# D-Robotics/hobot_stereonet

Hardware: AMD Instinct MI355X
Metric: stereo pairs/s at 1280x720 D=192 (ms/frame alongside) (higher is better)
Workload: dtype f16 (refinement-tower MFMA operands fp16 — 3x3 weights rounded per kernel so that every kernel's tap sum survives —, LeakyReLU applied after the fp16 rounding; low-resolution branch on 22-bit hi/lo split fp16 operands, 3 fp16 MFMAs per product in every 32-channel layer — profiles/r04_lowres_ablation

## Files before the change

hobot_stereonet_amd/api.py:

```python
from __future__ import annotations

import ctypes as C
import os
from typing import Optional

import numpy as np

from . import build as _build

SN_MEM_HOST, SN_MEM_DEVICE = 0, 1
PREC_DEFAULT, PREC_F16X3, PREC_F16, PREC_FP32, PREC_AUTO = 0, 1, 2, 3, 4
PREC_NAMES = {PREC_F16X3: "f16x3", PREC_F16: "f16", PREC_FP32: "fp32", PREC_AUTO: "auto"}
ABI_VERSION = 3
STAGES = ("features", "aggregate", "refine", "refine_conv", "total", "dominant")


class SnConfig(C.Structure):
    _fields_ = [("device", C.c_int), ("max_batch", C.c_int), ("width", C.c_int), ("height", C.c_int),
                ("dmax", C.c_int), ("precision", C.c_int), ("task_num", C.c_int), ("refine_chunk", C.c_int),
                ("piece", C.c_int)]


class SnIoInfo(C.Structure):
    _fields_ = [("width", C.c_int), ("height", C.c_int), ("dmax", C.c_int), ("in_channels", C.c_int),
                ("max_batch", C.c_int), ("precision", C.c_int), ("task_num", C.c_int), ("device", C.c_int),
                ("out_scale", C.c_float), ("in_bytes", C.c_size_t), ("out_bytes", C.c_size_t),
                ("flops_per_pair", C.c_double), ("refine_chunk", C.c_int), ("piece", C.c_int),
                ("tower_streams", C.c_int), ("refine_levels", C.c_int), ("precision_selected", C.c_int)]


class SnRefineStats(C.Structure):
    _fields_ = [("levels", C.c_int), ("precision", C.c_int), ("precision_selected", C.c_int), ("precision_last", C.c_int),
                ("calls", C.c_uint64), ("pairs", C.c_uint64), ("switches", C.c_uint64), ("reruns", C.c_uint64),
                ("level_px", C.c_double * 4), ("residual_px", C.c_double), ("running_px", C.c_double),
                ("envelope_px", C.c_double), ("limit_px", C.c_double), ("selfcheck_epe_px", C.c_double),
                ("selfcheck_residual_px", C.c_double)]


class SnAutoState(C.Structure):
    _fields_ = [("mode", C.c_int), ("calm", C.c_int), ("envelope_px", C.c_double), ("epe_per_px", C.c_double),
                ("running_px", C.c_double), ("switches", C.c_uint64)]


class StereoNetError(RuntimeError):
    def __init__(self, code: int, where: str, detail: str = ""):
        self.code = code
        super().__init__(f"{where}: {error_string(code)} (code {code}){': ' + detail if detail else ''}")


_lib = None


def load_library(path: Optional[str] = None):
    global _lib
    if _lib is not None:
        return _lib
    path = path or os.environ.get("STEREONET_HIP_LIB") or _build.LIB
    try:
        import torch
    except ImportError:
        pass
    if not os.path.exists(path) or (os.path.exists(_build.HIPCC) and _build.is_stale()):
        _build.build()
    lib = C.CDLL(path)
    vp, ip, i8p, i32p, fp, u8p = C.c_void_p, C.c_int, C.c_void_p, C.c_void_p, C.c_void_p, C.c_void_p
    lib.sn_create.argtypes = [C.c_char_p, C.POINTER(SnConfig), C.POINTER(vp)]
    lib.sn_destroy.argtypes = [vp]
    lib.sn_get_io_info.argtypes = [vp, C.POINTER(SnIoInfo)]
    lib.sn_strerror.restype = C.c_char_p
    lib.sn_strerror.argtypes = [ip]
    lib.sn_last_error.restype = C.c_char_p
    lib.sn_last_error.argtypes = [vp]
    lib.sn_infer_i8.argtypes = [vp, i8p, i32p, fp, ip, vp]
    lib.sn_infer_batch.argtypes = [vp, ip, i8p, i32p, fp, ip, vp]
    lib.sn_preprocess_nv12.argtypes = [vp, u8p, u8p, ip, ip, i8p, ip, vp]
    lib.sn_infer_sbs_nv12.argtypes = [vp, u8p, ip, ip, i32p, fp, i8p, ip, vp]
    lib.sn_preprocess_sbs_nv12_batch.argtypes = [vp, ip, u8p, ip, ip, i8p, ip, vp]
    lib.sn_submit.argtypes = [vp, i8p, i32p, fp, ip, C.POINTER(C.c_uint64)]
    lib.sn_submit_nv12.argtypes = [vp, u8p, ip, ip, i32p, fp, ip, C.POINTER(C.c_uint64)]
    lib.sn_wait.argtypes = [vp, C.c_uint64, C.POINTER(C.c_float)]
    lib.sn_synchronize.argtypes = [vp]
    lib.sn_set_profiling.argtypes = [vp, ip]
    lib.sn_get_stage_ms.argtypes = [vp, C.POINTER(C.c_float), ip]
    lib.sn_get_dominant_kernel.argtypes = [vp, C.c_char_p, C.c_size_t, C.POINTER(ip), C.POINTER(C.c_double),
                                           C.POINTER(C.c_double)]
    lib.sn_mgpu_shard.argtypes = [ip, ip, ip, C.POINTER(ip), C.POINTER(ip)]
    lib.sn_mgpu_create.argtypes = [C.c_char_p, C.POINTER(SnConfig), C.POINTER(ip), ip, C.POINTER(vp)]
    lib.sn_mgpu_destroy.argtypes = [vp]
    lib.sn_mgpu_get_info.argtypes = [vp, C.POINTER(ip), C.POINTER(ip), C.POINTER(ip)]
    lib.sn_mgpu_get_handle.argtypes = [vp, ip, C.POINTER(vp)]
    lib.sn_mgpu_infer_batch.argtypes = [vp, ip, i8p, i32p, fp]
    lib.sn_mgpu_infer_batch_device.argtypes = [vp, ip, C.POINTER(vp), i32p, fp]
    lib.sn_mgpu_submit_device.argtypes = [vp, ip, C.POINTER(vp), i32p, fp, C.POINTER(C.c_uint64)]
    lib.sn_mgpu_wait.argtypes = [vp, C.c_uint64]
    lib.sn_mgpu_ring_init.argtypes = [vp]
    lib.sn_mgpu_ring_submit.argtypes = [vp, C.POINTER(C.c_uint64), C.POINTER(ip)]
    lib.sn_mgpu_ring_wait.argtypes = [vp, C.c_uint64, C.POINTER(ip)]
    lib.sn_mgpu_last_error.restype = C.c_char_p
    lib.sn_mgpu_last_error.argtypes = [vp]
    lib.sn_dbg_conv2d.argtypes = [vp, fp, ip, ip, ip, fp, fp, ip, ip, ip, ip, fp, fp]
    lib.sn_dbg_down0.argtypes = [vp, i8p, ip, ip, fp, fp, ip, fp]
    lib.sn_dbg_compose_down01.argtypes = [fp, fp, fp, fp, fp, fp]
    lib.sn_dbg_round_kernels_f16.argtypes = [fp, ip, fp]
    lib.sn_dbg_down01.argtypes = [vp, i8p, ip, ip, fp, fp, fp, fp, fp]
    lib.sn_dbg_refin.argtypes = [vp, fp, i8p, ip, ip, ip, fp, fp, ip, fp]
    lib.sn_dbg_conv3d.argtypes = [vp, fp, ip, ip, ip, fp, fp, ip, fp]
    lib.sn_dbg_ref_conv_f16.argtypes = [vp, fp, ip, ip, fp, fp, ip, ip, fp, fp]
    lib.sn_dbg_ref_conv_f16x3.argtypes = [vp, fp, ip, ip, fp, fp, ip, ip, fp, fp]
    lib.sn_dbg_ref_block_f16.argtypes = [vp, fp, ip, ip, fp, fp, fp, fp, ip, fp]
    lib.sn_dbg_ref_block_f16x3.argtypes = [vp, fp, ip, ip, fp, fp, fp, fp, ip, ip, fp]
    lib.sn_dbg_ref_tail_f16.argtypes = [vp, ip, fp, ip, ip, fp, fp, fp, fp, fp, C.c_float, fp, ip, C.c_float, ip, ip, ip, fp, i32p]
    lib.sn_dbg_read.argtypes = [vp, C.c_char_p, fp, C.c_size_t, C.POINTER(C.c_size_t)]
    lib.sn_dbg_copy_limited.argtypes = [vp, vp, C.c_size_t, ip, vp]
    lib.sn_depth_from_raw.argtypes = [vp, ip, i32p, C.c_float, C.c_float, fp, fp, ip, vp]
    lib.sn_get_refine_stats.argtypes = [vp, C.POINTER(SnRefineStats)]
    lib.sn_auto_init.argtypes = [C.POINTER(SnAutoState), ip]
    lib.sn_auto_observe.argtypes = [C.POINTER(SnAutoState), C.c_double]
    lib.sn_auto_limit_px.argtypes = [C.POINTER(SnAutoState)]
    lib.sn_auto_limit_px.restype = C.c_double
    lib.sn_auto_envelope_px.argtypes = [ip]
    lib.sn_auto_envelope_px.restype = C.c_double
    for name in ("sn_create", "sn_destroy", "sn_get_io_info", "sn_infer_i8", "sn_infer_batch", "sn_preprocess_nv12",
                 "sn_infer_sbs_nv12", "sn_preprocess_sbs_nv12_batch", "sn_submit", "sn_submit_nv12", "sn_wait", "sn_synchronize", "sn_set_profiling",
                 "sn_get_stage_ms", "sn_get_dominant_kernel", "sn_mgpu_shard", "sn_mgpu_create", "sn_mgpu_destroy",
                 "sn_mgpu_get_info", "sn_mgpu_get_handle", "sn_mgpu_infer_batch", "sn_mgpu_infer_batch_device",
                 "sn_mgpu_submit_device", "sn_mgpu_wait", "sn_mgpu_ring_init", "sn_mgpu_ring_submit", "sn_mgpu_ring_wait", "sn_dbg_conv2d", "sn_dbg_down0", "sn_dbg_compose_down01", "sn_dbg_round_kernels_f16", "sn_dbg_down01", "sn_dbg_refin", "sn_dbg_conv3d", "sn_dbg_ref_conv_f16", "sn_dbg_ref_conv_f16x3", "sn_dbg_ref_block_f16", "sn_dbg_ref_block_f16x3", "sn_dbg_ref_tail_f16", "sn_dbg_read", "sn_dbg_copy_limited", "sn_depth_from_raw", "sn_get_refine_stats", "sn_auto_init", "sn_auto_observe"):
        getattr(lib, name).restype = C.c_int
    _lib = lib
    return lib


def round_kernels_f16(w):
    a = np.ascontiguousarray(w, np.float32)
    assert a.shape[-2:] == (3, 3)
    out = np.empty_like(a)
    rc = load_library().sn_dbg_round_kernels_f16(a.ctypes.data, a.size // 9, out.ctypes.data)
    if rc:
        raise StereoNetError(rc, "sn_dbg_round_kernels_f16")
    return out


def compose_down01(w0, b0, w1, b1):
    w0, b0, w1, b1 = (np.ascontiguousarray(a, np.float32) for a in (w0, b0, w1, b1))
    assert w0.shape == (32, 3, 5, 5) and w1.shape == (32, 32, 5, 5) and b0.shape == (32,) and b1.shape == (32,)
    weff = np.empty((9, 32, 3, 13, 13), np.float32)
    beff = np.empty((9, 32), np.float32)
    rc = load_library().sn_dbg_compose_down01(w0.ctypes.data, b0.ctypes.data, w1.ctypes.data, b1.ctypes.data,
                                              weff.ctypes.data, beff.ctypes.data)
    if rc:
        raise StereoNetError(rc, "sn_dbg_compose_down01")
    return weff, beff


def error_string(code: int) -> str:
    return load_library().sn_strerror(code).decode()


def _np_ptr(a: Optional[np.ndarray]):
    return a.ctypes.data if a is not None else None


class StereoNetHIP:

    def __init__(self, model_file: str, device: int = -1, max_batch: int = 1, width: int = 0, height: int = 0,
                 dmax: int = 0, precision: int = PREC_DEFAULT, task_num: int = 4, refine_chunk: int = 0,
                 piece: int = 0):
        self._lib = load_library()
        self._h = C.c_void_p()
        cfg = SnConfig(device, max_batch, width, height, dmax, precision, task_num, refine_chunk, piece)
        rc = self._lib.sn_create(model_file.encode(), C.byref(cfg), C.byref(self._h))
        if rc != 0:
            self._h = C.c_void_p()
            detail = self._lib.sn_last_error(None)
            raise StereoNetError(rc, f"sn_create({model_file!r})", detail.decode() if detail else "")
        info = SnIoInfo()
        self._check(self._lib.sn_get_io_info(self._h, C.byref(info)), "sn_get_io_info")
        self.info = info
        self.width, self.height, self.dmax = info.width, info.height, info.dmax
        self.max_batch = info.max_batch
        self.refine_chunk, self.piece, self.tower_streams = info.refine_chunk, info.piece, info.tower_streams
        self.refine_levels = info.refine_levels
        self.precision = info.precision
        self.out_scale = float(info.out_scale)
        self.flops_per_pair = float(info.flops_per_pair)

    def _check(self, rc: int, where: str):
        if rc != 0:
            detail = self._lib.sn_last_error(self._h).decode() if self._h else ""
            raise StereoNetError(rc, where, detail)

    def close(self):
        if getattr(self, "_h", None) and self._h.value:
            self._lib.sn_destroy(self._h)
            self._h = C.c_void_p()

    def __del__(self):
        try:
            self.close()
        except Exception:
            pass

    def __enter__(self):
        return self

    def __exit__(self, *exc):
        self.close()

    def refine_stats(self) -> dict:
        st = SnRefineStats()
        self._check(self._lib.sn_get_refine_stats(self._h, C.byref(st)), "sn_get_refine_stats")
        d = {k: getattr(st, k) for k, _ in SnRefineStats._fields_ if k != "level_px"}
        d["level_px"] = [float(v) for v in st.level_px][:max(1, st.levels)]
        for k in ("precision", "precision_selected", "precision_last"):
            d[k] = PREC_NAMES.get(d[k], str(d[k]))
        return d

    @property
    def precision_selected(self) -> int:
        info = SnIoInfo()
        self._check(self._lib.sn_get_io_info(self._h, C.byref(info)), "sn_get_io_info")
        return info.precision_selected

    def infer(self, in6: np.ndarray, want_disp: bool = True, want_raw: bool = True):
        x = np.ascontiguousarray(in6, dtype=np.int8)
        single = x.ndim == 3
        if single:
            x = x[None]
        n = x.shape[0]
        if x.shape[1:] != (6, self.height, self.width):
            raise StereoNetError(-1, "infer", f"input shape {x.shape} != (n,6,{self.height},{self.width})")
        disp = np.empty((n, self.height, self.width), np.float32) if want_disp else None
        raw = np.empty((n, self.height, self.width), np.int32) if want_raw else None
        self._check(self._lib.sn_infer_batch(self._h, n, x.ctypes.data, _np_ptr(raw), _np_ptr(disp), SN_MEM_HOST, None),
                    "sn_infer_batch")
        if single:
            return (disp[0] if disp is not None else None), (raw[0] if raw is not None else None)
        return disp, raw

    def infer_device(self, n: int, in_ptr: int, raw_ptr: int, disp_ptr: int, stream: int = 0):
        self._check(self._lib.sn_infer_batch(self._h, n, in_ptr, raw_ptr or None, disp_ptr or None, SN_MEM_DEVICE,
                                             stream or None), "sn_infer_batch")

    def preprocess_nv12(self, left: np.ndarray, right: np.ndarray, w: int, h: int) -> np.ndarray:
        left = np.ascontiguousarray(left, dtype=np.uint8)
        right = np.ascontiguousarray(right, dtype=np.uint8)
        out = np.empty((6, h, w), np.int8)
        self._check(self._lib.sn_preprocess_nv12(self._h, left.ctypes.data, right.ctypes.data, w, h, out.ctypes.data,
                                                 SN_MEM_HOST, None), "sn_preprocess_nv12")
        return out

    def preprocess_sbs_nv12_device(self, n: int, sbs_ptr: int, out_ptr: int, stream: int = 0):
        self._check(self._lib.sn_preprocess_sbs_nv12_batch(self._h, n, sbs_ptr, 2 * self.width, self.height, out_ptr,
                                                           SN_MEM_DEVICE, stream or None), "sn_preprocess_sbs_nv12_batch")

    def preprocess_sbs_nv12(self, sbs: np.ndarray) -> np.ndarray:
        x = np.ascontiguousarray(sbs, dtype=np.uint8).reshape(-1, 3 * self.width * self.height)
        out = np.empty((x.shape[0], 6, self.height, self.width), np.int8)
        self._check(self._lib.sn_preprocess_sbs_nv12_batch(self._h, x.shape[0], x.ctypes.data, 2 * self.width, self.height,
                                                           out.ctypes.data, SN_MEM_HOST, None), "sn_preprocess_sbs_nv12_batch")
        return out

    def infer_sbs_nv12(self, sbs: np.ndarray, want_tensor: bool = False):
        sbs = np.ascontiguousarray(sbs, dtype=np.uint8)
        disp = np.empty((self.height, self.width), np.float32)
        raw = np.empty((self.height, self.width), np.int32)
        ten = np.empty((6, self.height, self.width), np.int8) if want_tensor else None
        self._check(self._lib.sn_infer_sbs_nv12(self._h, sbs.ctypes.data, 2 * self.width, self.height, raw.ctypes.data,
                                                disp.ctypes.data, _np_ptr(ten), SN_MEM_HOST, None), "sn_infer_sbs_nv12")
        return (disp, raw, ten) if want_tensor else (disp, raw)

    def submit(self, in6: np.ndarray, raw_out: Optional[np.ndarray], disp_out: Optional[np.ndarray],
               timeout_ms: int = -1) -> int:
        x = np.ascontiguousarray(in6, dtype=np.int8)
        t = C.c_uint64()
        self._check(self._lib.sn_submit(self._h, x.ctypes.data, _np_ptr(raw_out), _np_ptr(disp_out), timeout_ms,
                                        C.byref(t)), "sn_submit")
        return t.value

    def submit_nv12(self, sbs: np.ndarray, raw_out: Optional[np.ndarray], disp_out: Optional[np.ndarray],
                    timeout_ms: int = -1) -> int:
        x = np.ascontiguousarray(sbs, dtype=np.uint8)
        if x.size != 3 * self.width * self.height:
            raise StereoNetError(-1, "submit_nv12", f"frame has {x.size} bytes, expected {3 * self.width * self.height}")
        t = C.c_uint64()
        self._check(self._lib.sn_submit_nv12(self._h, x.ctypes.data, 2 * self.width, self.height, _np_ptr(raw_out),
                                             _np_ptr(disp_out), timeout_ms, C.byref(t)), "sn_submit_nv12")
        return t.value

    def wait(self, ticket: int) -> float:
        ms = C.c_float()
        self._check(self._lib.sn_wait(self._h, ticket, C.byref(ms)), "sn_wait")
        return ms.value

    def depth_from_raw(self, raw: np.ndarray, focal_px: float = 527.1931762695312, baseline_mm: float = 119.89382172,
                       want_disp: bool = False):
        r = np.ascontiguousarray(raw, dtype=np.int32)
        if r.ndim not in (2, 3) or r.shape[-2:] != (self.height, self.width):
            raise StereoNetError(-1, "depth_from_raw", f"raw shape {r.shape} != ([n,] {self.height}, {self.width})")
        n = 1 if r.ndim == 2 else r.shape[0]
        if n < 1 or n > self.max_batch:
            raise StereoNetError(-1, "depth_from_raw", f"{n} maps, the engine was created for 1..{self.max_batch}")
        depth = np.empty(r.shape, np.float32)
        disp = np.empty(r.shape, np.float32) if want_disp else None
        self._check(self._lib.sn_depth_from_raw(self._h, n, r.ctypes.data, focal_px, baseline_mm, depth.ctypes.data,
                                                _np_ptr(disp), SN_MEM_HOST, None), "sn_depth_from_raw")
        return (depth, disp) if want_disp else depth

    def synchronize(self):
        self._check(self._lib.sn_synchronize(self._h), "sn_synchronize")

    def set_profiling(self, on: bool):
        self._check(self._lib.sn_set_profiling(self._h, int(on)), "sn_set_profiling")

    def stage_ms(self) -> dict:
        arr = (C.c_float * len(STAGES))()
        self._check(self._lib.sn_get_stage_ms(self._h, arr, len(STAGES)), "sn_get_stage_ms")
        return dict(zip(STAGES, [float(v) for v in arr]))

    def dominant_kernel(self) -> dict:
        name = C.create_string_buffer(128)
        launches = C.c_int()
        fl, by = C.c_double(), C.c_double()
        self._check(self._lib.sn_get_dominant_kernel(self._h, name, 128, C.byref(launches), C.byref(fl), C.byref(by)),
                    "sn_get_dominant_kernel")
        return {"name": name.value.decode(), "launches": launches.value, "flops_per_launch": fl.value,
                "bytes_per_launch": by.value}

    def dbg_conv2d(self, x, wt, bias, k, stride=1, dil=1, lrelu=False, residual=None, x3=False, slots=False, tower32=False, dma=False):
        x = np.ascontiguousarray(x, np.float32)
        wt = np.ascontiguousarray(wt, np.float32)
        bias = np.ascontiguousarray(bias, np.float32)
        cin, h, w = x.shape
        ho, wo = (h, w) if stride == 1 else (h // 2, w // 2)
        out = np.empty((32, ho, wo), np.float32)
        res = np.ascontiguousarray(residual, np.float32) if residual is not None else None
        self._check(self._lib.sn_dbg_conv2d(self._h, x.ctypes.data, cin, h, w, wt.ctypes.data, bias.ctypes.data, k,
                                            stride, dil, int(lrelu) | (2 if x3 else 0) | (4 if slots else 0) | (8 if tower32 else 0) | (16 if dma else 0), _np_ptr(res),
                                            out.ctypes.data),
                    "sn_dbg_conv2d")
        return out

    def dbg_down0(self, in6, wt, bias, tc=32):
        x = np.ascontiguousarray(in6, np.int8)
        wt = np.ascontiguousarray(wt, np.float32)
        bias = np.ascontiguousarray(bias, np.float32)
        _, h, w = x.shape
        ho, wo = (h + 15) // 16 * 8, (w + 15) // 16 * 8
        out = np.empty((2, 32, ho, wo), np.float32)
        self._check(self._lib.sn_dbg_down0(self._h, x.ctypes.data, h, w, wt.ctypes.data, bias.ctypes.data, tc,
                                           out.ctypes.data), "sn_dbg_down0")
        return out

    def dbg_down01(self, in6, w0, b0, w1, b1):
        x = np.ascontiguousarray(in6, np.int8)
        w0, b0, w1, b1 = (np.ascontiguousarray(a, np.float32) for a in (w0, b0, w1, b1))
        assert w0.shape == (32, 3, 5, 5) and w1.shape == (32, 32, 5, 5) and b0.shape == (32,) and b1.shape == (32,)
        _, h, w = x.shape
        ho, wo = (h + 15) // 16 * 4, (w + 15) // 16 * 4
        out = np.empty((2, 32, ho, wo), np.float32)
        self._check(self._lib.sn_dbg_down01(self._h, x.ctypes.data, h, w, w0.ctypes.data, b0.ctypes.data, w1.ctypes.data,
                                            b1.ctypes.data, out.ctypes.data), "sn_dbg_down01")
        return out

    def dbg_refin(self, disp_low, in6, dmax, wt, bias, split=False):
        x = np.ascontiguousarray(in6, np.int8)
        dl = np.ascontiguousarray(disp_low, np.float32)
        wt = np.ascontiguousarray(wt, np.float32)
        bias = np.ascontiguousarray(bias, np.float32)
        _, h, w = x.shape
        hp, wp = (h + 15) // 16 * 16, (w + 15) // 16 * 16
        assert dl.shape == (hp // 16, wp // 16)
        out = np.empty((32, hp, wp), np.float32)
        self._check(self._lib.sn_dbg_refin(self._h, dl.ctypes.data, x.ctypes.data, h, w, dmax, wt.ctypes.data,
                                           bias.ctypes.data, int(split), out.ctypes.data), "sn_dbg_refin")
        return out

    def dbg_conv3d(self, x, wt, bias, lrelu=False, x3=False, slots=False, dma=False):
        x = np.ascontiguousarray(x, np.float32)
        wt = np.ascontiguousarray(wt, np.float32)
        bias = np.ascontiguousarray(bias, np.float32)
        _, d, h, w = x.shape
        out = np.empty_like(x)
        self._check(self._lib.sn_dbg_conv3d(self._h, x.ctypes.data, d, h, w, wt.ctypes.data, bias.ctypes.data,
                                            int(lrelu) | (2 if x3 else 0) | (4 if slots else 0) | (8 if dma else 0), out.ctypes.data),
                    "sn_dbg_conv3d")
        return out

    def dbg_ref_conv_f16(self, x, wt, bias, dil=1, lrelu=False, residual=None, tile_w=0):
        x = np.ascontiguousarray(x, np.float32)
        wt = np.ascontiguousarray(wt, np.float32)
        bias = np.ascontiguousarray(bias, np.float32)
        _, h, w = x.shape
        out = np.empty((32, h, w), np.float32)
        res = np.ascontiguousarray(residual, np.float32) if residual is not None else None
        flags = int(bool(lrelu)) | (2 if tile_w == 64 else 4 if tile_w == 32 else 0)
        self._check(self._lib.sn_dbg_ref_conv_f16(self._h, x.ctypes.data, h, w, wt.ctypes.data, bias.ctypes.data, dil,
                                                  flags, _np_ptr(res), out.ctypes.data), "sn_dbg_ref_conv_f16")
        return out

    def dbg_ref_conv_f16x3(self, x, wt, bias, dil=1, lrelu=False, residual=None):
        x = np.ascontiguousarray(x, np.float32)
        wt = np.ascontiguousarray(wt, np.float32)
        bias = np.ascontiguousarray(bias, np.float32)
        _, h, w = x.shape
        out = np.empty((32, h, w), np.float32)
        res = np.ascontiguousarray(residual, np.float32) if residual is not None else None
        self._check(self._lib.sn_dbg_ref_conv_f16x3(self._h, x.ctypes.data, h, w, wt.ctypes.data, bias.ctypes.data, dil,
                                                    int(lrelu), _np_ptr(res), out.ctypes.data), "sn_dbg_ref_conv_f16x3")
        return out

    def dbg_ref_block_f16(self, x, w1, b1, w2, b2, dil=1, fused=0):
        dil = dil | (fused << 8)
        a = [np.ascontiguousarray(v, np.float32) for v in (x, w1, b1, w2, b2)]
        _, h, w = a[0].shape
        out = np.empty((32, h, w), np.float32)
        self._check(self._lib.sn_dbg_ref_block_f16(self._h, a[0].ctypes.data, h, w, a[1].ctypes.data, a[2].ctypes.data,
                                                   a[3].ctypes.data, a[4].ctypes.data, dil, out.ctypes.data),
                    "sn_dbg_ref_block_f16")
        return out

    def dbg_ref_block_f16x3(self, x, w1, b1, w2, b2, dil=1, streamed=False):
        a = [np.ascontiguousarray(v, np.float32) for v in (x, w1, b1, w2, b2)]
        _, h, w = a[0].shape
        out = np.empty((32, h, w), np.float32)
        self._check(self._lib.sn_dbg_ref_block_f16x3(self._h, a[0].ctypes.data, h, w, a[1].ctypes.data, a[2].ctypes.data,
                                                     a[3].ctypes.data, a[4].ctypes.data, dil, int(streamed), out.ctypes.data),
                    "sn_dbg_ref_block_f16x3")
        return out

    def dbg_ref_tail_f16(self, x, w1, b1, w2, b2, head_w, head_b, low, ups, dnorm, h_out, w_out, form):
        a = [np.ascontiguousarray(v, np.float32) for v in (x, w1, b1, w2, b2, head_w, low)]
        n, _, hk, wk = a[0].shape
        assert a[6].shape == (n, hk // ups, wk // ups)
        disp = np.empty((n, h_out, w_out), np.float32)
        raw = np.empty((n, h_out, w_out), np.int32)
        self._check(self._lib.sn_dbg_ref_tail_f16(self._h, n, a[0].ctypes.data, hk, wk, a[1].ctypes.data, a[2].ctypes.data,
                                                  a[3].ctypes.data, a[4].ctypes.data, a[5].ctypes.data, float(head_b),
                                                  a[6].ctypes.data, ups, float(dnorm), h_out, w_out, form, disp.ctypes.data,
                                                  raw.ctypes.data), "sn_dbg_ref_tail_f16")
        return disp, raw

    def stream_priority_high(self) -> bool:
        return bool(self.dbg_read("stream_prio")[0])

    def dbg_read(self, what: str) -> np.ndarray:
        n = C.c_size_t()
        self._check(self._lib.sn_dbg_read(self._h, what.encode(), None, 0, C.byref(n)), "sn_dbg_read")
        out = np.empty(n.value, np.float32)
        self._check(self._lib.sn_dbg_read(self._h, what.encode(), out.ctypes.data, n.value, C.byref(n)), "sn_dbg_read")
        return out


def mgpu_shard(n: int, ndev: int, k: int):
    lib = load_library()
    first, count = C.c_int(), C.c_int()
    rc = lib.sn_mgpu_shard(n, ndev, k, C.byref(first), C.byref(count))
    if rc != 0:
        raise StereoNetError(rc, "sn_mgpu_shard")
    return first.value, count.value


class SnMgpuRing(C.Structure):
    _fields_ = [("next", C.c_uint64), ("slot_ticket", C.c_uint64 * 2)]


class MgpuRing:

    def __init__(self):
        self._lib = load_library()
        self._r = SnMgpuRing()
        self._lib.sn_mgpu_ring_init(C.byref(self._r))

    def submit(self):
        t, s = C.c_uint64(), C.c_int()
        rc = self._lib.sn_mgpu_ring_submit(C.byref(self._r), C.byref(t), C.byref(s))
        if rc != 0:
            raise StereoNetError(rc, "sn_mgpu_ring_submit")
        return t.value, s.value

    def wait(self, ticket: int) -> int:
        s = C.c_int()
        rc = self._lib.sn_mgpu_ring_wait(C.byref(self._r), C.c_uint64(ticket), C.byref(s))
        if rc != 0:
            raise StereoNetError(rc, "sn_mgpu_ring_wait")
        return s.value


class StereoNetMultiGPU:

    def __init__(self, model_file: str, devices=None, ndev: int = 0, max_batch: int = 1, precision: int = PREC_DEFAULT,
                 refine_chunk: int = 0, piece: int = 0, width: int = 0, height: int = 0, dmax: int = 0):
        self._lib = load_library()
        self._m = C.c_void_p()
        devs = list(devices) if devices is not None else None
        if devs is None and ndev <= 0:
            import torch
            ndev = torch.cuda.device_count() if torch.cuda.is_available() else 0
            if ndev <= 0:
                raise StereoNetError(-4, "StereoNetMultiGPU: no GPU visible and neither devices nor ndev given")
        n = len(devs) if devs is not None else ndev
        arr = (C.c_int * n)(*devs) if devs is not None else None
        cfg = SnConfig(-1, max_batch, width, height, dmax, precision, 4, refine_chunk, piece)
        rc = self._lib.sn_mgpu_create(model_file.encode(), C.byref(cfg), arr, n, C.byref(self._m))
        if rc != 0:
            self._m = C.c_void_p()
            raise StereoNetError(rc, f"sn_mgpu_create({model_file!r}, ndev={n})")
        nd, per, kind = C.c_int(), C.c_int(), C.c_int()
        self._lib.sn_mgpu_get_info(self._m, C.byref(nd), C.byref(per), C.byref(kind))
        self.ndev, self.per_device_batch, self.gather_kind = nd.value, per.value, kind.value
        h = C.c_void_p()
        self._lib.sn_mgpu_get_handle(self._m, 0, C.byref(h))
        info = SnIoInfo()
        self._lib.sn_get_io_info(h, C.byref(info))
        self.width, self.height, self.dmax = info.width, info.height, info.dmax
        self.max_batch = max_batch

    def _check(self, rc: int, where: str):
        if rc != 0:
            raise StereoNetError(rc, where, self._lib.sn_mgpu_last_error(self._m).decode() if self._m else "")

    def engine_stream_priority_high(self, k: int = 0) -> bool:
        h = C.c_void_p()
        self._check(self._lib.sn_mgpu_get_handle(self._m, k, C.byref(h)), "sn_mgpu_get_handle")
        v, n = np.empty(1, np.float32), C.c_size_t()
        rc = self._lib.sn_dbg_read(h, b"stream_prio", v.ctypes.data, 1, C.byref(n))
        if rc != 0:
            raise StereoNetError(rc, "sn_dbg_read(stream_prio)")
        return bool(v[0])

    def infer(self, in6: np.ndarray):
        x = np.ascontiguousarray(in6, dtype=np.int8)
        n = x.shape[0]
        disp = np.empty((n, self.height, self.width), np.float32)
        raw = np.empty((n, self.height, self.width), np.int32)
        self._check(self._lib.sn_mgpu_infer_batch(self._m, n, x.ctypes.data, raw.ctypes.data, disp.ctypes.data),
                    "sn_mgpu_infer_batch")
        return disp, raw

    def infer_device(self, n: int, in_ptrs, raw_root_ptr: int, disp_root_ptr: int):
        arr = (C.c_void_p * self.ndev)(*[C.c_void_p(p) for p in in_ptrs])
        self._check(self._lib.sn_mgpu_infer_batch_device(self._m, n, arr, raw_root_ptr or None, disp_root_ptr or None),
                    "sn_mgpu_infer_batch_device")

    def submit_device(self, n: int, in_ptrs, raw_root_ptr: int, disp_root_ptr: int) -> int:
        arr = (C.c_void_p * self.ndev)(*[C.c_void_p(p) for p in in_ptrs])
        t = C.c_uint64()
        self._check(self._lib.sn_mgpu_submit_device(self._m, n, arr, raw_root_ptr or None, disp_root_ptr or None, C.byref(t)),
                    "sn_mgpu_submit_device")
        return t.value

    def wait(self, ticket: int):
        self._check(self._lib.sn_mgpu_wait(self._m, C.c_uint64(ticket)), "sn_mgpu_wait")

    def close(self):
        if getattr(self, "_m", None) and self._m.value:
            self._lib.sn_mgpu_destroy(self._m)
            self._m = C.c_void_p()

    def __enter__(self):
        return self

    def __exit__(self, *exc):
        self.close()

    def __del__(self):
        try:
            self.close()
        except Exception:
            pass
```

hobot_stereonet_amd/csrc/sn_stream_block.hpp:

```cpp
#pragma once

#ifdef SN_STREAM_TIMING
#define SN_STAMP(k)                                                                                   \
  do {                                                                                                \
    if (blockIdx.x == 17 && q >= 8 && q < 24) {                                                       \
      const unsigned long long t_ = __builtin_readcyclecounter();                                     \
      if (lane == 0) reinterpret_cast<unsigned long long*>(dump + 64)[(wave * 16 + q - 8) * 8 + (k)] = t_; \
    }                                                                                                 \
  } while (0)
#define SN_STAMP_WG(k)                                                                                          \
  do {                                                                                                          \
    if (threadIdx.x == 0) {                                                                                     \
      unsigned long long* d_ = reinterpret_cast<unsigned long long*>(dump + 64) + 1152 + 4 * blockIdx.x + (k);  \
      d_[0] = __builtin_readcyclecounter();                                                                     \
      d_[2] = wall_clock64();                                                                                   \
    }                                                                                                           \
  } while (0)
#else
#define SN_STAMP(k) do { } while (0)
#define SN_STAMP_WG(k) do { } while (0)
#endif

namespace sn {

template <int DIL_, int TW_ = 64, int R_ = 4, int NXS_ = 6, int NWR_ = 4, bool HEAD_ = false>
struct StreamTile {
  static constexpr bool HEAD = HEAD_;
  static constexpr int DIL = DIL_, TW = TW_, R = R_, NXS = NXS_, NTS = 3, PF = NXS_ - (HEAD_ ? 3 : 4);
  static constexpr int NWR = NWR_;
  static constexpr int HS = HEAD_ ? 1 : 0;
  static constexpr int YW = TW - 2 * DIL;
  static constexpr int OW = YW - 2 * HS;
  static constexpr int X0OFF = -HS;
  static constexpr int LAG = HEAD_ ? 3 : 2;
  static constexpr int PROWS = 2 * R + 2;
  static constexpr int PRING_BYTES = HEAD_ ? PROWS * 9 * TW * 4 : 0;
  static constexpr int WIN_BYTES = HEAD_ ? NWR_ * 2 * 64 * 4 : 0;
  static constexpr int XW = TW + 2 * DIL;
  static constexpr int CSEG = TW / 32;
  static constexpr int SPW = R * CSEG / NWR;
  static constexpr int XROW = 4 * XW, TROW = 4 * TW;
  static constexpr int XGROUP = R * XROW;
  static constexpr int NINST = (XGROUP + 63) / 64;
  static constexpr int KW = (NINST + NWR - 1) / NWR;
  static constexpr int XGP = NINST * 64;
  static constexpr int TGP = R * TROW;
  static constexpr int XRING = NXS * XGP;
  static constexpr int TRING = NTS * TGP + 64;
  static constexpr int LDS_BYTES = (XRING + TRING) * 16 + 2 * 2 * 16 * 4 + PRING_BYTES + WIN_BYTES;
  static constexpr int ROWS_ABOVE = (R + HS) * DIL, ROWS_BELOW = (R + 2 + HS) * DIL - 1;
  static_assert(!HEAD_ || (DIL_ == 1 && R_ == 4 && TW_ == 64 && NWR_ == 4), "the tail form is written for the dilation-1 strip shape");
  static_assert(SPW == 1 || SPW == 2, "segments per wave");
  static_assert(CSEG % SPW == 0, "a wave's segments lie in one row");
  static_assert(PF == 2, "prefetch distance the counted waits are written for");
  static_assert(R == 4 || R == 2, "rows per step");
  static_assert(LDS_BYTES <= 160 * 1024, "one workgroup per CU");
};

struct StreamSched {
  int nstrips;
  int hsub;
  int total_rows;
  int rows_per_wg;
};

template <int R, int HS = 0>
struct StreamIter {
  int f, f_end, hsub;
  int sp, v0, v1, n, j, live;
  __device__ __forceinline__ void next_unit() {
    if (f >= f_end) { live = 0; return; }
    sp = f / hsub;
    v0 = f - sp * hsub;
    int L = hsub - v0;
    if (L > f_end - f) L = f_end - f;
    v1 = v0 + L;
    n = (L + 2 + 2 * HS + R - 1) / R;
    j = 0;
    f += L;
    live = 1;
  }
  __device__ __forceinline__ void step(int q, int lag, int f0, int f1, int hsub_) {
    if (q < lag) { live = 0; return; }
    if (q == lag) { f = f0; f_end = f1; hsub = hsub_; next_unit(); return; }
    if (live && ++j > n) next_unit();
  }
};

__device__ __forceinline__ unsigned lrelu_pack2(float a, float b) { return act_pack2_f16(a, b, (_Float16)kSlope); }

template <int HI>
__device__ __forceinline__ float res_add(unsigned r, float acc) {
  float d;
  if (HI) asm("v_fma_mix_f32 %0, %1, 1.0, %2 op_sel:[1,0,0] op_sel_hi:[1,0,0]" : "=v"(d) : "v"(r), "v"(acc));
  else asm("v_fma_mix_f32 %0, %1, 1.0, %2 op_sel_hi:[1,0,0]" : "=v"(d) : "v"(r), "v"(acc));
  return d;
}

__device__ __forceinline__ unsigned lds_addr(const void* p) {
  return (unsigned)(size_t)(const __attribute__((address_space(3))) void*)p;
}

template <int DIL, int COLW, int SPW>
__device__ __forceinline__ void stream_conv36(const uint4* const (&rp)[3], const half8 (&wf)[18], const f32x16& bv,
                                              f32x16 (&acc)[SPW]) {
  constexpr int NB = 3 * SPW;
  half8 b[2][NB];
  auto fetch = [&](int batch, half8 (&dst)[NB]) {
    const int kk = batch / 3, ky = batch - kk * 3;
#pragma unroll
    for (int kx = 0; kx < 3; ++kx)
#pragma unroll
      for (int s = 0; s < SPW; ++s)
        dst[kx * SPW + s] = *reinterpret_cast<const half8*>(rp[ky] + (2 * kk * COLW + s * 32 + kx * DIL));
  };
  fetch(0, b[0]);
#pragma unroll
  for (int batch = 0; batch < 6; ++batch) {
    if (batch + 1 < 6) fetch(batch + 1, b[(batch + 1) & 1]);
    const int kk = batch / 3, ky = batch - kk * 3;
#pragma unroll
    for (int kx = 0; kx < 3; ++kx)
#pragma unroll
      for (int s = 0; s < SPW; ++s) {
        const int tap = ky * 3 + kx;
        if (batch == 0 && kx == 0) acc[s] = __builtin_amdgcn_mfma_f32_32x32x16_f16(wf[tap * 2 + kk], b[0][s], bv, 0, 0, 0);
        else acc[s] = __builtin_amdgcn_mfma_f32_32x32x16_f16(wf[tap * 2 + kk], b[batch & 1][kx * SPW + s], acc[s], 0, 0, 0);
      }
  }
  constexpr int AHEAD = SPW == 2 ? 8 : 5, NM = 18 * SPW;
  __builtin_amdgcn_sched_group_barrier(0x100, 4 + AHEAD, 0);
#pragma unroll
  for (int i = 0; i < NM - AHEAD; ++i) {
    __builtin_amdgcn_sched_group_barrier(0x008, 1, 0);
    __builtin_amdgcn_sched_group_barrier(0x100, 1, 0);
  }
  __builtin_amdgcn_sched_group_barrier(0x008, AHEAD, 0);
}

__device__ __forceinline__ void glds16(unsigned lds_dst, unsigned voff, const void* base) {
  unsigned keep;
  asm volatile(
      "s_mov_b32 %0, m0\n\t"
      "s_mov_b32 m0, %1\n\t"
      "s_nop 0\n\t"
      "global_load_lds_dwordx4 %2, %3\n\t"
      "s_mov_b32 m0, %0"
      : "=&s"(keep)
      : "s"(lds_dst), "v"(voff), "s"(base)
      : "memory");
}

__device__ __forceinline__ void glds4(unsigned lds_dst, unsigned voff, const void* base) {
  unsigned keep;
  asm volatile(
      "s_mov_b32 %0, m0\n\t"
      "s_mov_b32 m0, %1\n\t"
      "s_nop 0\n\t"
      "global_load_lds_dword %2, %3\n\t"
      "s_mov_b32 m0, %0"
      : "=&s"(keep)
      : "s"(lds_dst), "v"(voff), "s"(base)
      : "memory");
}

struct StreamHeadArgs {
  const float* w;
  const float* disp_low;
  float* out_disp;
  int32_t* out_raw;
  float bias, dmax, inv_q;
  int hl, wl, H, W;
  UpScale ups;
  unsigned long long* stat = nullptr;
};

template <int DIL, int TW, int R, int NXS, int NWR, bool HEAD = false>
__global__ __launch_bounds__(128 * NWR, NWR / 2) __attribute__((amdgpu_waves_per_eu(NWR / 2, NWR / 2))) void k_ref_block_stream_f16(const uint4* __restrict__ xin, uint4* __restrict__ yout,
                                                                const uint4* __restrict__ wfrag1, const float* __restrict__ bias1,
                                                                const uint4* __restrict__ wfrag2, const float* __restrict__ bias2,
                                                                RefGeom g, StreamSched sc, uint4* __restrict__ dump, StreamHeadArgs ha) {
  using T = StreamTile<DIL, TW, R, NXS, NWR, HEAD>;
  constexpr int HS = T::HS;
  extern __shared__ __attribute__((aligned(16))) uint4 lds[];
  uint4* const xring = lds;
  uint4* const tring = lds + T::XRING;
  float* const s_bias = reinterpret_cast<float*>(tring + T::TRING);
  float* const pring = s_bias + 64;
  float* const s_win = pring + T::PRING_BYTES / 4;
  const int tid = threadIdx.x, lane = tid & 63;
  const int wave = __builtin_amdgcn_readfirstlane(tid >> 6);
  const int j = lane & 31, gh = lane >> 5;
  const int role = wave / NWR, rw = wave % NWR;

  const int f0 = (int)blockIdx.x * sc.rows_per_wg;
  int f1 = f0 + sc.rows_per_wg;
  if (f1 > sc.total_rows) f1 = sc.total_rows;
  if (f0 >= f1) return;
  SN_STAMP_WG(0);
  int nss = T::LAG;
  for (int f = f0; f < f1;) {
    const int v0 = f % sc.hsub;
    int L = sc.hsub - v0;
    if (L > f1 - f) L = f1 - f;
    nss += (L + 2 + 2 * HS + R - 1) / R + 1;
    f += L;
  }
  auto decode_sp = [&](int sp, int& img, int& py, int& x0) {
    const int t = sp / sc.nstrips;
    x0 = (sp - t * sc.nstrips) * T::OW + T::X0OFF;
    img = t / DIL;
    py = t - img * DIL;
  };
  const unsigned plane_b = (unsigned)g.Hs * (unsigned)g.Ws * 16u;

  half8 wf[18];
  {
    const uint4* wsrc = role ? wfrag2 : wfrag1;
#pragma unroll
    for (int i = 0; i < 18; ++i) {
      const uint4 a = wsrc[i * 64 + lane];
      wf[i] = *reinterpret_cast<const half8*>(&a);
    }
    if (tid < 64) {
      const int c = tid >> 5, g2 = (tid >> 4) & 1, r = tid & 15;
      s_bias[tid] = (c ? bias2 : bias1)[(r & 3) + 8 * (r >> 2) + 4 * g2];
    }
#pragma unroll
    for (int i = 0; i < 18; ++i) asm volatile("" : "+v"(wf[i]));
    asm volatile("s_waitcnt vmcnt(0) lgkmcnt(0)" ::: "memory");
  }



  const int seg0 = rw * T::SPW;
  const int rowW = seg0 / T::CSEG;
  const int cseg0 = seg0 % T::CSEG;

  if (role == 0) {
    const int lane_x = gh * T::XW + cseg0 * 32 + j;
    const int lane_w = cseg0 * 32 + j;
    constexpr int KWMAX = T::KW;
    const int kw = (T::NINST - rw + NWR - 1) / NWR;
    unsigned dma_voff[KWMAX];
#pragma unroll
    for (int k = 0; k < KWMAX; ++k) {
      const int i = rw + NWR * k;
      int s = i * 64 + lane;
      s = s < T::XGROUP ? s : T::XGROUP - 1;
      const int r = s / T::XROW;
      const int rem = s - r * T::XROW;
      const int blk = rem / T::XW;
      const int c = rem - blk * T::XW;
      dma_voff[k] = (unsigned)blk * plane_b + ((unsigned)(r * DIL) * (unsigned)g.Ws + (unsigned)c) * 16u;
    }
    long last_base = 0;
    auto dma_issue = [&](const StreamIter<R, HS>& it, int grp) {
      if (it.live) {
        int img, py, x0;
        decode_sp(it.sp, img, py, x0);
        const int row = (it.v0 - HS - R + R * it.j) * DIL + py;
        last_base = (((long)img * 4 * g.Hs + (row + kRefPad)) * (long)g.Ws + (x0 - 2 * DIL + kRefPad)) * 16;
      }
      const char* src = reinterpret_cast<const char*>(xin) + last_base;
      const unsigned dst = lds_addr(xring + grp * T::XGP);
#pragma unroll
      for (int k = 0; k < KWMAX; ++k)
        if (k < kw) glds16(dst + (unsigned)(rw + NWR * k) * 1024u, dma_voff[k], src);
    };
    auto wait_group = [&](auto extra) {
      constexpr int E = decltype(extra)::value;
      if (kw == KWMAX) wait_vmcnt<KWMAX + E>();
      else wait_vmcnt<KWMAX - 1 + E>();
    };
    StreamIter<R, HS> dm, c1, fin, fin2;
    dm.live = c1.live = fin.live = fin2.live = 0;
    int fin_img = 0, fin_x0 = 0, fin2_img = 0, fin2_x0 = 0;
    auto win_first_col = [&](int xs) {
      float sx = ((float)xs + 0.5f) * ha.ups.rs - 0.5f;
      sx = sx < 0.f ? 0.f : sx;
      return (int)sx;
    };
    int p4 = 0;
    float moved = 0.f;
    dm.step(0, 0, f0, f1, sc.hsub);
    dma_issue(dm, 0);
    dm.step(1, 0, f0, f1, sc.hsub);
    dma_issue(dm, 1);
    wait_group(std::integral_constant<int, 0>{});
    block_barrier();

    int c1_py = 0, c1_x0 = 0;
    int qx = 0, qt = 0;
    for (int q = 0; q < nss; ++q) {
      dm.step(q + 2, 0, f0, f1, sc.hsub);
      c1.step(q, 0, f0, f1, sc.hsub);
      const int do1 = c1.live && c1.j >= 1;
      const int gx0 = qx, gx1 = qx >= 1 ? qx - 1 : qx - 1 + NXS;
      const int gxp = qx + 2 >= NXS ? qx + 2 - NXS : qx + 2;
      SN_STAMP(0);
      if constexpr (HEAD) {
        fin.step(q, 3, f0, f1, sc.hsub);
        if (fin.live && fin.j >= 1) {
          if (fin.j == 1) {
            int py;
            decode_sp(fin.sp, fin_img, py, fin_x0);
          }
          const int o = fin.v0 - 4 + R * (fin.j - 1) + rowW;
          if (o >= fin.v0 && o < fin.v1 && o < ha.H) {
            const int pb = p4 + 8 >= T::PROWS ? p4 + 8 - T::PROWS : p4 + 8;
            float acc = ha.bias;
#pragma unroll
            for (int ky = 0; ky < 3; ++ky) {
              int pr = pb + rowW - 2 + ky;
              pr = pr < 0 ? pr + T::PROWS : (pr >= T::PROWS ? pr - T::PROWS : pr);
              const float* prow = pring + pr * (9 * TW) + lane - 1;
#pragma unroll
              for (int kx = 0; kx < 3; ++kx) acc += prow[(ky * 3 + kx) * TW + kx];
            }
            const int X = fin_x0 + lane;
            float sy = ((float)o + 0.5f) * ha.ups.rs - 0.5f;
            float sx = ((float)X + 0.5f) * ha.ups.rs - 0.5f;
            sy = sy < 0.f ? 0.f : sy;
            sx = sx < 0.f ? 0.f : sx;
            const int y0 = (int)sy, x0 = (int)sx;
            const int x1 = x0 < ha.wl - 1 ? x0 + 1 : x0;
            const float ly = sy - (float)y0, lx = sx - (float)x0;
            const float hy = 1.0f - ly, hx = 1.0f - lx;
            const int cb = win_first_col(fin_x0);
            const float* w0 = s_win + rw * 128;
            const float v = hy * (hx * w0[x0 - cb] + lx * w0[x1 - cb]) + ly * (hx * w0[64 + x0 - cb] + lx * w0[64 + x1 - cb]);
            const float up = v * ha.ups.mul;
            float d = up + ha.dmax * acc;
            const float mv = fabsf(ha.dmax * acc);
            d = d > 0.f ? d : 0.f;
            if (lane >= 1 && lane <= T::OW && X < ha.W) {
              moved += mv;
              const size_t oi = ((size_t)fin_img * ha.H + o) * ha.W + X;
              if (ha.out_disp) ha.out_disp[oi] = d;
              if (ha.out_raw) ha.out_raw[oi] = (int32_t)__float2int_rn(d * ha.inv_q);
            }
          }
        }
      }
      if constexpr (HEAD) {
        fin2.step(q, 2, f0, f1, sc.hsub);
        if (fin2.live && fin2.j >= 1) {
          if (fin2.j == 1) {
            int py;
            decode_sp(fin2.sp, fin2_img, py, fin2_x0);
          }
          const int o = fin2.v0 - 4 + R * (fin2.j - 1) + rowW;
          if (o >= fin2.v0 && o < fin2.v1 && o < ha.H) {
            float sy = ((float)o + 0.5f) * ha.ups.rs - 0.5f;
            sy = sy < 0.f ? 0.f : sy;
            const int y0 = (int)sy;
            const int y1 = y0 < ha.hl - 1 ? y0 + 1 : y0;
            int c = win_first_col(fin2_x0) + lane;
            c = c < ha.wl - 1 ? c : ha.wl - 1;
            const float* lowp = ha.disp_low + (size_t)fin2_img * ha.hl * ha.wl;
            const unsigned dst = lds_addr(s_win + rw * 128);
            asm volatile("s_waitcnt lgkmcnt(0)" ::: "memory");
            glds4(dst, (unsigned)c * 4u, lowp + (size_t)y0 * ha.wl);
            glds4(dst + 256u, (unsigned)c * 4u, lowp + (size_t)y1 * ha.wl);
          }
        }
      }
      dma_issue(dm, gxp);
      SN_STAMP(1);
      if (do1) {
        if (c1.j == 1) {
          int img;
          decode_sp(c1.sp, img, c1_py, c1_x0);
        }
        const uint4* xp[3];
#pragma unroll
        for (int ky = 0; ky < 3; ++ky) {
          const int rr = rowW - 2 + ky;
          xp[ky] = xring + (rr < 0 ? gx1 : gx0) * T::XGP + (rr & (R - 1)) * T::XROW + lane_x;
        }
        const f32x16 bv = *reinterpret_cast<const f32x16*>(s_bias + gh * 16);
        f32x16 acc[T::SPW];
        stream_conv36<DIL, T::XW, T::SPW>(xp, wf, bv, acc);
        SN_STAMP(2);
        const int trow = (c1.v0 - HS - 1 + R * (c1.j - 1) + rowW) * DIL + c1_py;
        const bool row_ok = trow >= 0 && trow < g.H;
        const int tc0 = c1_x0 - DIL;
        const bool interior = row_ok && tc0 >= 0 && tc0 + TW <= g.W;
        uint4* tw = tring + qt * T::TGP + rowW * T::TROW + lane_w;
        auto write_t = [&](auto is_interior) {
#pragma unroll
          for (int s = 0; s < T::SPW; ++s) {
            bool inside = true;
            if (!decltype(is_interior)::value) {
              const int c = tc0 + (cseg0 + s) * 32 + j;
              inside = row_ok && c >= 0 && c < g.W;
            }
            unsigned pk[4][2];
#pragma unroll
            for (int qd = 0; qd < 4; ++qd)
#pragma unroll
              for (int hp = 0; hp < 2; ++hp) {
                const unsigned u = lrelu_pack2(acc[s][4 * qd + 2 * hp], acc[s][4 * qd + 2 * hp + 1]);
                pk[qd][hp] = (decltype(is_interior)::value || inside) ? u : 0u;
              }
#pragma unroll
            for (int qd = 0; qd < 4; ++qd)
              *reinterpret_cast<uint2*>(reinterpret_cast<char*>(tw + qd * T::TW + s * 32) + gh * 8) = uint2{pk[qd][0], pk[qd][1]};
          }
        };
        if (interior) write_t(std::true_type{});
        else write_t(std::false_type{});
      }
      SN_STAMP(3);
      wait_group(std::integral_constant<int, 0>{});
      asm volatile("s_waitcnt lgkmcnt(0)" ::: "memory");
      SN_STAMP(4);
      block_barrier();
      qx = qx + 1 == NXS ? 0 : qx + 1;
      qt = qt + 1 == T::NTS ? 0 : qt + 1;
      p4 = p4 + R >= T::PROWS ? p4 + R - T::PROWS : p4 + R;
    }
    if constexpr (HEAD) refine_stat_commit(ha.stat, moved);
    SN_STAMP_WG(1);
  } else {
    const int lane_t = gh * T::TW + cseg0 * 32 + j;
    const int lane_y = 2 * DIL + cseg0 * 32 + j;
    block_barrier();

    StreamIter<R, HS> c2, ep;
    c2.live = ep.live = 0;
    half8 ah[2], al[2];
    uint2 rres[T::SPW][4];
    int p4 = 0;
    if constexpr (HEAD) {
#pragma unroll
      for (int kk = 0; kk < 2; ++kk)
#pragma unroll
        for (int e = 0; e < 8; ++e) {
          const float wv = j < 9 ? ha.w[(16 * kk + 8 * gh + e) * 9 + j] : 0.f;
          const _Float16 hi = (_Float16)wv;
          ah[kk][e] = hi;
          al[kk][e] = (_Float16)((wv - (float)hi) * kSplitScale);
        }
#pragma unroll
      for (int s = 0; s < T::SPW; ++s)
#pragma unroll
        for (int qd = 0; qd < 4; ++qd) rres[s][qd] = uint2{0u, 0u};
    }
    int ep_img = 0, ep_py = 0, ep_x0 = 0;
    const unsigned lane_o = (unsigned)(cseg0 * 32 + j) * 16u + (unsigned)(2 * gh) * plane_b;
    f32x16 acc[T::SPW];
#pragma unroll
    for (int s = 0; s < T::SPW; ++s)
#pragma unroll
      for (int r = 0; r < 16; ++r) acc[s][r] = 0.f;
    int qx = 0, qt = 0;
    for (int q = 0; q < nss; ++q) {
      c2.step(q, 1, f0, f1, sc.hsub);
      ep.step(q, 2, f0, f1, sc.hsub);
      const int do2 = c2.live && c2.j >= 1;
      const int doe = ep.live && ep.j >= 1;
      const int gx2 = qx >= 2 ? qx - 2 : qx - 2 + NXS, gx3 = qx >= 3 ? qx - 3 : qx - 3 + NXS;
      const int gt1 = qt >= 1 ? qt - 1 : qt - 1 + T::NTS, gt2 = qt >= 2 ? qt - 2 : qt - 2 + T::NTS;
      SN_STAMP(0);
      if (doe) {
        if (ep.j == 1) decode_sp(ep.sp, ep_img, ep_py, ep_x0);
        const int sub = ep.v0 - HS - 2 + R * (ep.j - 1) + rowW;
        const int row = sub * DIL + ep_py;
        if constexpr (HEAD) {
          const bool row_ok = row >= 0 && row < g.H;
          const bool interior = row_ok && ep_x0 >= 0 && ep_x0 + TW <= g.W;
          int prow = p4 + 2 + rowW;
          prow = prow >= T::PROWS ? prow - T::PROWS : prow;
#pragma unroll
          for (int s = 0; s < T::SPW; ++s) {
            const int col = ep_x0 + (cseg0 + s) * 32 + j;
            const bool ok = row_ok && col >= 0 && col < g.W;
            unsigned pk[4][2];
#pragma unroll
            for (int qd = 0; qd < 4; ++qd) {
              const half4 rv = *reinterpret_cast<const half4*>(&rres[s][qd]);
              const uint2 rw2 = *reinterpret_cast<const uint2*>(&rv);
              pk[qd][0] = lrelu_pack2(res_add<0>(rw2.x, acc[s][4 * qd]), res_add<1>(rw2.x, acc[s][4 * qd + 1]));
              pk[qd][1] = lrelu_pack2(res_add<0>(rw2.y, acc[s][4 * qd + 2]), res_add<1>(rw2.y, acc[s][4 * qd + 3]));
            }
            if (!interior) {
#pragma unroll
              for (int qd = 0; qd < 4; ++qd) {
                pk[qd][0] = ok ? pk[qd][0] : 0u;
                pk[qd][1] = ok ? pk[qd][1] : 0u;
              }
            }
            f32x16 a0, a1;
#pragma unroll
            for (int r = 0; r < 16; ++r) {
              a0[r] = 0.f;
              a1[r] = 0.f;
            }
#pragma unroll
            for (int kk = 0; kk < 2; ++kk) {
              const auto r0 = __builtin_amdgcn_permlane32_swap(pk[2 * kk][0], pk[2 * kk + 1][0], false, false);
              const auto r1 = __builtin_amdgcn_permlane32_swap(pk[2 * kk][1], pk[2 * kk + 1][1], false, false);
              const uint4 sl = uint4{r0[0], r1[0], r0[1], r1[1]};
              const half8 xh = *reinterpret_cast<const half8*>(&sl);
              a0 = __builtin_amdgcn_mfma_f32_32x32x16_f16(ah[kk], xh, a0, 0, 0, 0);
              a1 = __builtin_amdgcn_mfma_f32_32x32x16_f16(al[kk], xh, a1, 0, 0, 0);
            }
            float* dst = pring + prow * (9 * TW) + (cseg0 + s) * 32 + j;
#pragma unroll
            for (int r = 0; r < 4; ++r) dst[(4 * gh + r) * TW] = a0[r] + a1[r] * kSplitInv;
            if (gh == 0) dst[8 * TW] = a0[4] + a1[4] * kSplitInv;
          }
        } else
        if (sub >= ep.v0 && sub < ep.v1 && row < g.H) {
          const int rr = rowW - 2;
          const uint4* xrow = xring + (rr < 0 ? gx3 : gx2) * T::XGP + (rr & (R - 1)) * T::XROW + lane_y;
          const unsigned ob = (((unsigned)ep_img * 4u * (unsigned)g.Hs + (unsigned)(row + kRefPad)) * (unsigned)g.Ws +
                               (unsigned)(ep_x0 + kRefPad)) * 16u;
#pragma unroll
          for (int s = 0; s < T::SPW; ++s) {
            unsigned pk[4][2];
#pragma unroll
            for (int qd = 0; qd < 4; ++qd) {
              const half4 rv = *reinterpret_cast<const half4*>(reinterpret_cast<const char*>(xrow + qd * T::XW + s * 32) + gh * 8);
              const uint2 rw2 = *reinterpret_cast<const uint2*>(&rv);
              pk[qd][0] = lrelu_pack2(res_add<0>(rw2.x, acc[s][4 * qd]), res_add<1>(rw2.x, acc[s][4 * qd + 1]));
              pk[qd][1] = lrelu_pack2(res_add<0>(rw2.y, acc[s][4 * qd + 2]), res_add<1>(rw2.y, acc[s][4 * qd + 3]));
            }
            uint4 sl[2];
#pragma unroll
            for (int k = 0; k < 2; ++k) {
              const auto r0 = __builtin_amdgcn_permlane32_swap(pk[k][0], pk[k + 2][0], false, false);
              const auto r1 = __builtin_amdgcn_permlane32_swap(pk[k][1], pk[k + 2][1], false, false);
              sl[k] = uint4{r0[0], r1[0], r0[1], r1[1]};
            }
            const int c = (cseg0 + s) * 32 + j;
            if (c < T::OW && ep_x0 + c < g.W) {
#pragma unroll
              for (int k = 0; k < 2; ++k) {
                char* o = reinterpret_cast<char*>(yout) + (ob + (unsigned)k * plane_b + (unsigned)s * 512u);
                *reinterpret_cast<uint4*>(o + lane_o) = sl[k];
              }
            }
          }
        }
      }
      SN_STAMP(1);
      if (do2) {
        if constexpr (HEAD) {
          const int rr = rowW - 2;
          const int gx1 = qx >= 1 ? qx - 1 : qx - 1 + NXS;
          const uint4* xrow = xring + (rr < 0 ? gx2 : gx1) * T::XGP + (rr & (R - 1)) * T::XROW + lane_y;
#pragma unroll
          for (int s = 0; s < T::SPW; ++s)
#pragma unroll
            for (int qd = 0; qd < 4; ++qd)
              rres[s][qd] = *reinterpret_cast<const uint2*>(reinterpret_cast<const char*>(xrow + qd * T::XW + s * 32) + gh * 8);
        }
        const uint4* tp[3];
#pragma unroll
        for (int ky = 0; ky < 3; ++ky) {
          const int rr = rowW - 2 + ky;
          tp[ky] = tring + (rr < 0 ? gt2 : gt1) * T::TGP + (rr & (R - 1)) * T::TROW + lane_t;
        }
        const f32x16 bv = *reinterpret_cast<const f32x16*>(s_bias + (2 + gh) * 16);
        stream_conv36<DIL, T::TW, T::SPW>(tp, wf, bv, acc);
      }
      SN_STAMP(2);
      asm volatile("s_waitcnt lgkmcnt(0)" ::: "memory");
      SN_STAMP(3);
      block_barrier();
      qx = qx + 1 == NXS ? 0 : qx + 1;
      qt = qt + 1 == T::NTS ? 0 : qt + 1;
      p4 = p4 + R >= T::PROWS ? p4 + R - T::PROWS : p4 + R;
    }
  }
}

}
```

hobot_stereonet_amd/csrc/stereonet_hip.hip:

```cpp
#include <hip/hip_runtime.h>

#include <algorithm>

#include <atomic>
#include <chrono>
#include <cmath>
#include <condition_variable>
#include <cstdio>
#include <cstdlib>
#include <cstring>
#include <mutex>
#include <string>
#include <unordered_map>
#include <vector>

#ifndef SN_DIAGNOSTICS
#define SN_DIAGNOSTICS 0
#endif

#include "../../include/stereonet_hip.h"
#include "sn_internal.h"
#include "sn_kernels.hpp"

namespace {
// ... 460 lines not shown
#else
unsigned ablate_mask(const char* var) {
  const char* e = getenv(var);
  if (!e || !*e) return 0u;
  if (!strcmp(e, "all")) return (1u << kAblCount) - 1u;
  unsigned m = 0;
  std::string str(e);
  size_t pos = 0;
  while (pos <= str.size()) {
    size_t c = str.find(',', pos);
    if (c == std::string::npos) c = str.size();
    const std::string t = str.substr(pos, c - pos);
    int idx = -1;
    if (t.rfind("down", 0) == 0 && t.size() == 5 && t[4] >= '1' && t[4] <= '3') idx = kAblDown + (t[4] - '1');
    else if (t.rfind("agg", 0) == 0 && t.size() == 4 && t[3] >= '0' && t[3] <= '3') idx = kAblAgg + (t[3] - '0');
    else if (t.size() >= 2 && t[0] == 'f' && atoi(t.c_str() + 1) >= 0 && atoi(t.c_str() + 1) <= 12 && isdigit((unsigned char)t[1])) idx = kAblFeat + atoi(t.c_str() + 1);
    if (idx >= 0) m |= 1u << idx;
    pos = c + 1;
  }
  return m;
}

__global__ void k_zero_lo_slots(uint4* t, size_t hw, size_t nblk) {
  const size_t total = nblk * hw;
  for (size_t i = (size_t)blockIdx.x * 256 + threadIdx.x; i < total; i += (size_t)gridDim.x * 256) {
    const size_t b = i / hw, r = i - b * hw;
    t[(2 * b + 1) * hw + r] = uint4{0u, 0u, 0u, 0u};
  }
}
inline hipError_t zero_lo_slots(hipStream_t st, float* tensor, int nimg, size_t hw) {
  hipLaunchKernelGGL(k_zero_lo_slots, dim3(1024), dim3(256), 0, st, reinterpret_cast<uint4*>(tensor), hw, (size_t)nimg * 4);
  return hipGetLastError();
}
#endif

bool agg_dma_enabled() {
  static const bool on = [] {
    const char* e = getenv("SN_AGG_DMA");
    return !(e && *e == '0') && ablate_mask("SN_ABLATE_X") == 0;
  }();
  return on;
}

VolPad vol_pad(int Dl, int hl, int wl) { return VolPad{Dl, hl, wl, VolPad::ph(hl), VolPad::pw(wl)}; }

template <bool OUTSLOT, bool HEADP = false>
hipError_t launch_agg_dma(hipStream_t st, const ConvLayer& L, const uint4* vin, const VolPad& g, int npairs, void* out,
                          bool lrelu, int num_cu, const uint4* head_frag = nullptr) {
  ConvArgs a{};
  a.wpk = reinterpret_cast<const float*>(L.wx3);
  a.bias = L.bias;
  a.out = reinterpret_cast<float*>(out);
  a.res = reinterpret_cast<const float*>(head_frag);
  if (HEADP != (head_frag != nullptr)) return hipErrorInvalidValue;
  a.nimg = npairs * g.Dl;
  a.cin_pad = L.cin_pad;
  a.Ho = g.H;
  a.Wo = g.W;
  a.dil = 1;
  a.pad = 1;
  a.lrelu = lrelu ? 1 : 0;
  a.tiles_x = (g.W + 15) / 16;
  a.tiles_y = (g.H + 7) / 8;
  auto kern = k_agg_x3s_dma<OUTSLOT, HEADP>;
  hipError_t e = ensure_lds_attr(kern, (int)AggDma::LDS_BYTES);
  if (e != hipSuccess) return e;
  const int total = a.tiles_x * a.tiles_y * a.nimg;
  int blocks = num_cu;
  if (blocks > (total + 7) / 8 * 8) blocks = (total + 7) / 8 * 8;
  blocks = (blocks + 7) / 8 * 8;
  hipLaunchKernelGGL(kern, dim3(blocks), dim3(256), AggDma::LDS_BYTES, st, a, vin, g);
  return hipGetLastError();
}

bool feat_dma_enabled() {
  static const bool on = [] {
    const char* e = getenv("SN_FEAT_DMA");
    return !(e && *e == '0') && ablate_mask("SN_ABLATE_X") == 0;
  }();
  return on;
}

FeatPad feat_pad(int H, int W) { return FeatPad{H, W, FeatPad::ph(H), FeatPad::pw(W)}; }

template <bool OUTSLOT, bool HASRES>
hipError_t launch_feat_dma(hipStream_t st, const ConvLayer& L, const uint4* vin, const FeatPad& g, int nimg, void* out,
                           const void* res, bool lrelu, int num_cu) {
  ConvArgs a{};
  a.wpk = reinterpret_cast<const float*>(L.wx3);
  a.bias = L.bias;
  a.out = reinterpret_cast<float*>(out);
  a.res = reinterpret_cast<const float*>(res);
  a.nimg = nimg;
  a.cin_pad = L.cin_pad;
  a.Ho = g.H;
  a.Wo = g.W;
  a.dil = 1;
  a.pad = 1;
  a.lrelu = lrelu ? 1 : 0;
  a.tiles_x = (g.W + 15) / 16;
  a.tiles_y = (g.H + 7) / 8;
  auto kern = k_feat_x3s_dma<OUTSLOT, HASRES>;
  hipError_t e = ensure_lds_attr(kern, (int)FeatDma::LDS_BYTES);
  if (e != hipSuccess) return e;
  const int total = a.tiles_x * a.tiles_y * a.nimg;
  int blocks = 2 * num_cu;
  if (blocks > (total + 7) / 8 * 8) blocks = (total + 7) / 8 * 8;
  blocks = (blocks + 7) / 8 * 8;
  hipLaunchKernelGGL(kern, dim3(blocks), dim3(256), FeatDma::LDS_BYTES, st, a, vin, g);
  return hipGetLastError();
}

bool down_dma_enabled() {
  static const bool on = [] {
    const char* e = getenv("SN_DOWN_DMA");
    return !(e && *e == '0') && ablate_mask("SN_ABLATE_X") == 0;
  }();
  return on;
}

SlotGeom down_in_geom(int Ho, int Wo) { return SlotGeom{DownDma::ph(Ho), DownDma::pw(Wo), DownDma::PADY, DownDma::PADX}; }

hipError_t launch_down_dma(hipStream_t st, const ConvLayer& L, const uint4* vin, int nimg, int Ho, int Wo, void* out,
                           const SlotGeom& go, bool lrelu, int num_cu) {
  ConvArgs a{};
  a.wpk = reinterpret_cast<const float*>(L.wx3);
  a.bias = L.bias;
  a.out = reinterpret_cast<float*>(out);
  a.res = nullptr;
  a.nimg = nimg;
  a.cin_pad = L.cin_pad;
  a.Ho = Ho;
  a.Wo = Wo;
  a.dil = 1;
  a.pad = 2;
  a.lrelu = lrelu ? 1 : 0;
  a.tiles_x = (Wo + DownDma::TC - 1) / DownDma::TC;
  a.tiles_y = (Ho + DownDma::TR - 1) / DownDma::TR;
  hipError_t e = ensure_lds_attr(k_down_x3s_dma, (int)DownDma::LDS_BYTES);
  if (e != hipSuccess) return e;
  const int total = a.tiles_x * a.tiles_y * nimg;
  int blocks = num_cu;
  if (blocks > (total + 7) / 8 * 8) blocks = (total + 7) / 8 * 8;
  blocks = (blocks + 7) / 8 * 8;
  hipLaunchKernelGGL(k_down_x3s_dma, dim3(blocks), dim3(256), DownDma::LDS_BYTES, st, a, vin, down_in_geom(Ho, Wo), go);
  return hipGetLastError();
}

int upload_head(sn_handle* h, const HostLayer& l, HeadLayer* out) {
  HIP_TRY(h, dalloc(&out->w, (size_t)kC * l.taps));
  HIP_TRY(h, hipMemcpy(out->w, l.w, (size_t)kC * l.taps * sizeof(float), hipMemcpyHostToDevice));
  out->bias = l.b[0];
  return SN_OK;
}

int upload_agg_head_frag(sn_handle* h, const HostLayer& l, HeadLayer* out) {
  std::vector<_Float16> pk((size_t)2 * 2 * 64 * 8, (_Float16)0.f);
  for (int kk = 0; kk < 2; ++kk)
    for (int lane = 0; lane < 64; ++lane)
      for (int e = 0; e < 8; ++e) {
        const int m = lane & 31, c = 16 * kk + 8 * (lane >> 5) + e;
        if (m >= 27) continue;
        const float w = l.w[(size_t)c * 27 + m];
        const _Float16 hi = (_Float16)w;
        const size_t base = ((size_t)(2 * kk) * 64 + lane) * 8 + e;
        pk[base] = hi;
        pk[base + 64 * 8] = (_Float16)((w - (float)hi) * kSplitScale);
      }
  HIP_TRY(h, dalloc(&out->pfrag, pk.size() / 8));
  HIP_TRY(h, hipMemcpy(out->pfrag, pk.data(), pk.size() * sizeof(_Float16), hipMemcpyHostToDevice));
  return SN_OK;
}

bool head_fold_enabled() {
  static const bool on = !(getenv("SN_HEAD_FOLD") != nullptr && atoi(getenv("SN_HEAD_FOLD")) == 0);
  return on;
}

template <class K>
hipError_t ensure_lds_attr(K kern, int bytes) {
  static std::mutex mu;
  static std::unordered_map<const void*, unsigned long long> done;
  int dev = 0;
  if (hipGetDevice(&dev) != hipSuccess) dev = 0;
  const unsigned long long bit = 1ull << (dev & 63);
  const void* key = reinterpret_cast<const void*>(kern);
  std::lock_guard<std::mutex> lk(mu);
  unsigned long long& m = done[key];
  if (m & bit) return hipSuccess;
  const hipError_t e = hipFuncSetAttribute(key, hipFuncAttributeMaxDynamicSharedMemorySize, bytes);
  if (e == hipSuccess) m |= bit;
  return e;
}

template <int KS, int STRIDE, int DIL, int CH, int TR, int TC, class Loader, bool PF = true, int MINW = 1>
hipError_t launch_conv(hipStream_t st, const ConvLayer& L, const Loader& ld, int nimg, int Ho, int Wo,
                       float* out, const float* res, bool lrelu) {
  constexpr int dil = DIL;
  ConvArgs a{};
  a.wpk = L.wpk;
  a.bias = L.bias;
  a.out = out;
  a.res = res;
  a.nimg = nimg;
  a.cin_pad = L.cin_pad;
  a.Ho = Ho;
  a.Wo = Wo;
  a.dil = dil;
  a.pad = (KS / 2) * dil;
  a.lrelu = lrelu ? 1 : 0;
  a.tiles_x = (Wo + TC - 1) / TC;
  a.tiles_y = (Ho + TR - 1) / TR;
  const int rows_in = (TR - 1) * STRIDE + (KS - 1) * dil + 1;
  const int cols_in = (TC - 1) * STRIDE + (KS - 1) * dil + 1;
  const int pitch = STRIDE == 1 ? cols_in : 2 * ((cols_in + 1) / 2);
  const size_t lds = ((size_t)CH * KS * KS * 32 + (size_t)CH * rows_in * pitch) * sizeof(float);
  auto kern = k_conv_c32_mfma<KS, STRIDE, DIL, CH, TR, TC, Loader, PF, MINW>;
  if (lds > 64 * 1024) {
    hipError_t e = ensure_lds_attr(kern, (int)lds);
    if (e != hipSuccess) return e;
  }
  const int nwg = a.tiles_x * a.tiles_y * nimg;
  hipLaunchKernelGGL(kern, dim3(nwg), dim3(256), lds, st, a, ld);
  return hipGetLastError();
}

template <int DIL>
hipError_t conv3x3_d(hipStream_t st, const ConvLayer& L, const float* in, int nimg, int H, int W, float* out,
                     const float* res, bool lrelu) {
  LoadF32 ld{in, kC, H, W};
  if (H * W <= 64 * 128) return launch_conv<3, 1, DIL, 8, 4, 32>(st, L, ld, nimg, H, W, out, res, lrelu);
  if (DIL >= 4) return launch_conv<3, 1, DIL, 4, 16, 64>(st, L, ld, nimg, H, W, out, res, lrelu);
  return launch_conv<3, 1, DIL, 8, 8, 64>(st, L, ld, nimg, H, W, out, res, lrelu);
}

template <int DIL, int CPH, int NW = 8>
hipError_t launch_ref_conv_f32(hipStream_t st, const ConvLayer& L, const float* in, int nimg, int H, int W, float* out,
                               const float* res, bool lrelu, int num_cu) {
  using T = F32Tile<DIL, CPH, 64, NW>;
  auto kern = res ? k_ref_conv_f32<DIL, CPH, true, NW> : k_ref_conv_f32<DIL, CPH, false, NW>;
  if (T::LDS_BYTES > 64 * 1024 - 1024) {
    hipError_t e = ensure_lds_attr(kern, T::LDS_BYTES);
    if (e != hipSuccess) return e;
  }
  const int total = ((W + T::TW - 1) / T::TW) * ((H + T::TH - 1) / T::TH) * nimg;
  int grid = 2 * total < num_cu ? 2 * total : num_cu;
  static const int grid_env = getenv("SN_F32_GRID") ? atoi(getenv("SN_F32_GRID")) : 0;
  if (grid_env > 0) grid = grid_env < 2 * total ? grid_env : 2 * total;
  if (grid < 1) grid = 1;
  hipLaunchKernelGGL(kern, dim3(grid), dim3(64 * NW), T::LDS_BYTES, st, in, out, res, L.wpk, L.bias, nimg, H, W, lrelu ? 1 : 0);
  return hipGetLastError();
}

inline bool f32_tower_env() {
  static const bool on = !(getenv("SN_F32_TOWER") != nullptr && atoi(getenv("SN_F32_TOWER")) == 0);
  return on;
}

hipError_t conv3x3(hipStream_t st, const ConvLayer& L, const float* in, int nimg, int H, int W, int dil,
                   float* out, const float* res, bool lrelu, int tower_cu = 0) {
  if (tower_cu > 0 && L.cin == kC && L.cin_pad == kC && (W & 3) == 0 && f32_tower_env()) {
    switch (dil) {
      case 1: return launch_ref_conv_f32<1, 8>(st, L, in, nimg, H, W, out, res, lrelu, tower_cu);
      case 2: return launch_ref_conv_f32<2, 8>(st, L, in, nimg, H, W, out, res, lrelu, tower_cu);
      case 4: return launch_ref_conv_f32<4, 4, 16>(st, L, in, nimg, H, W, out, res, lrelu, tower_cu);
      case 8: return launch_ref_conv_f32<8, 4, 16>(st, L, in, nimg, H, W, out, res, lrelu, tower_cu);
      default: return hipErrorInvalidValue;
    }
  }
  switch (dil) {
    case 1: return conv3x3_d<1>(st, L, in, nimg, H, W, out, res, lrelu);
    case 2: return conv3x3_d<2>(st, L, in, nimg, H, W, out, res, lrelu);
    case 4: return conv3x3_d<4>(st, L, in, nimg, H, W, out, res, lrelu);
    case 8: return conv3x3_d<8>(st, L, in, nimg, H, W, out, res, lrelu);
    default: return hipErrorInvalidValue;
  }
}

hipError_t conv5x5s2(hipStream_t st, const ConvLayer& L, const float* in, int nimg, int Hin, int Win,
                     float* out) {
  LoadF32 ld{in, kC, Hin, Win};
  const int Ho = Hin / 2, Wo = Win / 2;
  const long big_tiles = (long)((Wo + 63) / 64) * ((Ho + 7) / 8) * nimg;
  if (Ho * Wo <= 64 * 128 || big_tiles < 512) return launch_conv<5, 2, 1, 4, 4, 32>(st, L, ld, nimg, Ho, Wo, out, nullptr, false);
  return launch_conv<5, 2, 1, 4, 8, 64>(st, L, ld, nimg, Ho, Wo, out, nullptr, false);
}

RefGeom make_ref_geom(int Hp, int Wp) {
  RefGeom g{};
  g.tiles_x = (Wp + 63) / 64;
  g.tiles_y = (Hp + 7) / 8;
  g.H = Hp;
  g.W = Wp;
  g.Hs = (Hp + 15) / 16 * 16 + 2 * kRefPad;
  g.Ws = g.tiles_x * 64 + 2 * kRefPad;
  return g;
}

size_t ref16_slots(const RefGeom& g, int nimg) { return (size_t)nimg * 4 * g.Hs * g.Ws; }
using StreamTile1 = StreamTile<1, 64, 4, 6, 4>;
using StreamTile2 = StreamTile<2, 64, 4, 6, 4>;
using StreamTile4 = StreamTile<4, 128, 2, 6, 4>;
using StreamTile8 = StreamTile<8, 128, 2, 6, 4>;
using StreamTileTail = StreamTile<1, 64, 4, 5, 4, true>;
static_assert(StreamTileTail::ROWS_ABOVE <= kRefPad && StreamTileTail::ROWS_BELOW <= StreamTile8::ROWS_BELOW, "tail form stays inside the zero rows");
constexpr int cmax4(int a, int b, int c, int d) { return (a > b ? a : b) > (c > d ? c : d) ? (a > b ? a : b) : (c > d ? c : d); }
constexpr int kStreamRowsAbove = cmax4(StreamTile1::ROWS_ABOVE, StreamTile2::ROWS_ABOVE, StreamTile4::ROWS_ABOVE, StreamTile8::ROWS_ABOVE);
constexpr int kStreamRowsBelow = cmax4(StreamTile1::ROWS_BELOW, StreamTile2::ROWS_BELOW, StreamTile4::ROWS_BELOW, StreamTile8::ROWS_BELOW);
constexpr int kRefSlackRows = kStreamRowsBelow - kRefPad + 1;
constexpr int kRefFrontRows = (kStreamRowsAbove > kRefPad ? kStreamRowsAbove - kRefPad : 0) + 1;
static_assert(kRefSlackRows == 24 && kRefFrontRows == 9, "zero rows around the fp16 tower tensors follow the StreamTile list");
size_t ref_slack(const RefGeom& g) {
  const size_t rows = (size_t)kRefSlackRows * g.Ws;
  return rows > 4096 ? rows : 4096;
}
size_t ref_front(const RefGeom& g) { return (size_t)kRefFrontRows * g.Ws; }
hipError_t alloc_ref16(const RefGeom& g, size_t tensor_and_slack_slots, uint4** raw, uint4** base) {
  const size_t front = ref_front(g), all = front + tensor_and_slack_slots;
  hipError_t e = dalloc(raw, all);
  if (e != hipSuccess) return e;
  e = memset_now(*raw, 0, all * sizeof(uint4));
  *base = *raw + front;
  return e;
}

inline _Float16 f16_neighbour(_Float16 hval, bool up) {
  uint16_t b;
  memcpy(&b, &hval, 2);
  if (up) {
    if (b == 0x8000) b = 0x0001;
    else if (b & 0x8000) b -= 1;
    else b += 1;
  } else {
    if (b == 0x0000) b = 0x8001;
    else if (b & 0x8000) b += 1;
    else b -= 1;
  }
  _Float16 r;
  memcpy(&r, &b, 2);
  return r;
}

void round_kernel_sum_preserving(const float* w, _Float16* q) {
  double lo[9], hi[9];
  _Float16 hlo[9], hhi[9];
  for (int t = 0; t < 9; ++t) {
    const _Float16 n = (_Float16)w[t];
    const double nd = (double)n, wd = (double)w[t];
    hlo[t] = nd <= wd ? n : f16_neighbour(n, false);
    hhi[t] = nd >= wd ? n : f16_neighbour(n, true);
    lo[t] = (double)hlo[t] - wd;
    hi[t] = (double)hhi[t] - wd;
  }
  int best = 0;
  double best_score = 1e300;
  for (int m = 0; m < 512; ++m) {
    double sum = 0, sq = 0;
    for (int t = 0; t < 9; ++t) {
      const double e = (m >> t) & 1 ? hi[t] : lo[t];
      sum += e;
      sq += e * e;
    }
    const double score = std::fabs(sum) + 1e-3 * std::sqrt(sq);
    if (score < best_score) {
      best_score = score;
      best = m;
    }
  }
  for (int t = 0; t < 9; ++t) q[t] = (best >> t) & 1 ? hhi[t] : hlo[t];
}

bool w_round_sum_preserving() {
  const char* e = getenv("SN_W_ROUND");
  return !(e && strcmp(e, "rne") == 0);
}

int upload_ref_f16(sn_handle* h, const HostLayer& l, RefLayerF16* out) {
  std::vector<_Float16> q((size_t)kC * kC * 9);
  const bool sp = w_round_sum_preserving();
  for (size_t k = 0; k < (size_t)kC * kC; ++k) {
    if (sp) {
      round_kernel_sum_preserving(l.w + k * 9, &q[k * 9]);
    } else {
      for (int t = 0; t < 9; ++t) q[k * 9 + t] = (_Float16)l.w[k * 9 + t];
    }
  }
  std::vector<_Float16> pk((size_t)18 * 64 * 8);
  for (int tap = 0; tap < 9; ++tap)
    for (int kk = 0; kk < 2; ++kk)
      for (int lane = 0; lane < 64; ++lane)
        for (int e = 0; e < 8; ++e) {
          const int co = lane & 31, ci = 16 * kk + 8 * (lane >> 5) + e;
          pk[(((size_t)tap * 2 + kk) * 64 + lane) * 8 + e] = q[((size_t)co * kC + ci) * 9 + tap];
        }
  HIP_TRY(h, dalloc(&out->wfrag, (size_t)18 * 64));
  HIP_TRY(h, dalloc(&out->bias, kC));
  HIP_TRY(h, hipMemcpy(out->wfrag, pk.data(), pk.size() * sizeof(_Float16), hipMemcpyHostToDevice));
  HIP_TRY(h, hipMemcpy(out->bias, l.b, kC * sizeof(float), hipMemcpyHostToDevice));
  return SN_OK;
}

int upload_ref_f16x3(sn_handle* h, const HostLayer& l, RefLayerF16* out) {
  std::vector<_Float16> pk((size_t)36 * 64 * 8);
  for (int tap = 0; tap < 9; ++tap)
    for (int kk = 0; kk < 2; ++kk)
      for (int lane = 0; lane < 64; ++lane)
        for (int e = 0; e < 8; ++e) {
          const int co = lane & 31, ci = 16 * kk + 8 * (lane >> 5) + e;
          const float w = l.w[((size_t)co * kC + ci) * 9 + tap];
          const _Float16 hi = (_Float16)w;
          const size_t i = (((size_t)tap * 2 + kk) * 64 + lane) * 8 + e;
          pk[i] = hi;
          pk[(size_t)18 * 64 * 8 + i] = (_Float16)((w - (float)hi) * kSplitScale);
        }
  HIP_TRY(h, dalloc(&out->wfrag, (size_t)36 * 64));
  HIP_TRY(h, dalloc(&out->bias, kC));
  HIP_TRY(h, hipMemcpy(out->wfrag, pk.data(), pk.size() * sizeof(_Float16), hipMemcpyHostToDevice));
  HIP_TRY(h, hipMemcpy(out->bias, l.b, kC * sizeof(float), hipMemcpyHostToDevice));
  return SN_OK;
}

template <int DIL, int TW, int NBUF>
hipError_t launch_ref_f16x3(hipStream_t st, const RefLayerF16& L, const RefGeom& g, int num_cu, const uint4* in,
                            uint4* out, const uint4* res, size_t lo_slots, int nimg, bool lrelu) {
  using T = RefTile2<DIL, TW>;
  constexpr int lds_bytes = NBUF * 2 * T::BUF * 16;
  auto kern = res ? k_ref_conv_f16x3<DIL, TW, NBUF, true> : k_ref_conv_f16x3<DIL, TW, NBUF, false>;
  hipError_t e = ensure_lds_attr(kern, lds_bytes);
  if (e != hipSuccess) return e;
  RefGeom gt = g;
  gt.tiles_x = (g.W + TW - 1) / TW;
  const int total = gt.tiles_x * gt.tiles_y * nimg;
  const int band = (total + 7) / 8;
  int cap = num_cu / 8;
  if (cap < 1) cap = 1;
  const int rounds = (band + cap - 1) / cap;
  const int nlb = (band + rounds - 1) / rounds;
  hipLaunchKernelGGL(kern, dim3(nlb * 8), dim3(256), lds_bytes, st, in, out, res, lo_slots, L.wfrag, L.bias, gt, nimg,
                     lrelu ? 1 : 0);
  return hipGetLastError();
}

hipError_t ref_conv_f16x3(hipStream_t st, const RefLayerF16& L, const RefGeom& g, int num_cu, int dil, const uint4* in,
                          uint4* out, const uint4* res, size_t lo_slots, int nimg, bool lrelu) {
  switch (dil) {
    case 1: return launch_ref_f16x3<1, 64, 3>(st, L, g, num_cu, in, out, res, lo_slots, nimg, lrelu);
    case 2: return launch_ref_f16x3<2, 64, 3>(st, L, g, num_cu, in, out, res, lo_slots, nimg, lrelu);
    case 4: return launch_ref_f16x3<4, 32, 3>(st, L, g, num_cu, in, out, res, lo_slots, nimg, lrelu);
    case 8: return launch_ref_f16x3<8, 32, 2>(st, L, g, num_cu, in, out, res, lo_slots, nimg, lrelu);
    default: return hipErrorInvalidValue;
  }
}

template <int DIL, int TW, int NB = 3>
hipError_t launch_ref_f16_v2(hipStream_t st, const RefLayerF16& L, const RefGeom& g, int num_cu, const uint4* in,
                             uint4* out, const uint4* res, int nimg, bool lrelu, unsigned* tile_ctr) {
  using T = RefTile2<DIL, TW, 8, NB>;
  auto kern = res ? k_ref_conv_f16_v2<DIL, TW, true, 8, 2, NB> : k_ref_conv_f16_v2<DIL, TW, false, 8, 2, NB>;
  if (tile_ctr == nullptr) return hipErrorInvalidValue;
  if (T::LDS_BYTES > 64 * 1024) {
    hipError_t e = ensure_lds_attr(kern, T::LDS_BYTES);
    if (e != hipSuccess) return e;
  }
  static_assert(2 * T::LDS_BYTES <= 160 * 1024, "two tower workgroups per CU");
  RefGeom gt = g;
  gt.tiles_x = (g.W + TW - 1) / TW;
  gt.tiles_y = (g.H + 7) / 8;
  const int total = gt.tiles_x * gt.tiles_y * nimg;
  const int band = (total + 7) / 8;
  int cap = num_cu * 2 / 8;
  if (cap < 1) cap = 1;
  const int nlb = cap < band ? cap : band;
  hipLaunchKernelGGL(kern, dim3(nlb * 8), dim3(256), T::LDS_BYTES, st, in, out, res, L.wfrag, L.bias, gt, nimg,
                     lrelu ? 1 : 0, tile_ctr);
  return hipGetLastError();
}

template <class T>
hipError_t launch_ref_block_stream(hipStream_t st, const RefLayerF16& L1, const RefLayerF16& L2, const RefGeom& g, int num_cu,
                                   const uint4* x, uint4* y, int nimg, unsigned* dump, const StreamHeadArgs& ha = StreamHeadArgs{}) {
  constexpr int DIL = T::DIL;
  auto kern = k_ref_block_stream_f16<T::DIL, T::TW, T::R, T::NXS, T::NWR, T::HEAD>;
  if (dump == nullptr) return hipErrorInvalidValue;
  hipError_t e = ensure_lds_attr(kern, T::LDS_BYTES);
  if (e != hipSuccess) return e;
  StreamSched sc;
  const int Wn = T::HEAD ? ha.W : g.W, Hn = T::HEAD ? ha.H : g.H;
  if (T::HEAD && (!ha.w || !ha.disp_low || (!ha.out_disp && !ha.out_raw) || ha.W > g.W || ha.H > g.H || ha.ups.rs > 0.5f)) return hipErrorInvalidValue;
  sc.nstrips = (Wn + T::OW - 1) / T::OW;
  sc.hsub = (Hn + DIL - 1) / DIL;
  sc.total_rows = nimg * DIL * sc.nstrips * sc.hsub;
  static const int wg_env = getenv("SN_STREAM_WGS") ? atoi(getenv("SN_STREAM_WGS")) : 0;
  int nwg = wg_env > 0 ? wg_env : num_cu;
  if (nwg > sc.total_rows) nwg = sc.total_rows;
  if (nwg < 1) nwg = 1;
  sc.rows_per_wg = (sc.total_rows + nwg - 1) / nwg;
  const int grid = (sc.total_rows + sc.rows_per_wg - 1) / sc.rows_per_wg;
  hipLaunchKernelGGL(kern, dim3(grid), dim3(512), T::LDS_BYTES, st, x, y, L1.wfrag, L1.bias, L2.wfrag, L2.bias, g, sc,
                     reinterpret_cast<uint4*>(dump), ha);
  return hipGetLastError();
}

hipError_t ref_block_stream_tail(hipStream_t st, const RefLayerF16& L1, const RefLayerF16& L2, const RefGeom& g, int num_cu,
                                 const uint4* x, int nimg, unsigned* dump, const StreamHeadArgs& ha) {
  return launch_ref_block_stream<StreamTileTail>(st, L1, L2, g, num_cu, x, nullptr, nimg, dump, ha);
}

hipError_t ref_block_stream(hipStream_t st, const RefLayerF16& L1, const RefLayerF16& L2, const RefGeom& g, int num_cu, int dil,
                            const uint4* x, uint4* y, int nimg, unsigned* dump) {
  switch (dil) {
    case 1: return launch_ref_block_stream<StreamTile1>(st, L1, L2, g, num_cu, x, y, nimg, dump);
    case 2: return launch_ref_block_stream<StreamTile2>(st, L1, L2, g, num_cu, x, y, nimg, dump);
    case 4: return launch_ref_block_stream<StreamTile4>(st, L1, L2, g, num_cu, x, y, nimg, dump);
    case 8: return launch_ref_block_stream<StreamTile8>(st, L1, L2, g, num_cu, x, y, nimg, dump);
    default: return hipErrorInvalidValue;
  }
}
inline bool stream_block_supports(int dil) {
  static const int max_dil = getenv("SN_STREAM_DIL") ? atoi(getenv("SN_STREAM_DIL")) : 8;
  return (dil == 1 || dil == 2 || dil == 4 || dil == 8) && dil <= max_dil;
}

hipError_t launch_head_final_f16(hipStream_t st, bool split, const uint4* x, size_t lo_slots, const RefGeom& g,
                                 const float* w, float bias, const float* disp_low, int hl, int wl, int H, int W, float dmax,
                                 float inv_q, UpScale ups, float* out_disp, int32_t* out_raw, int nimg,
                                 unsigned long long* stat = nullptr) {
  constexpr int TH = 16;
  using T = HeadTile<TH>;
  const int tiles_x = (W + T::TWO - 1) / T::TWO, tiles_y = (H + TH - 1) / TH;
  const dim3 grid((unsigned)(tiles_x * tiles_y * nimg));
  if (split)
    hipLaunchKernelGGL((k_head_final_f16<true, TH>), grid, dim3(256), T::LDS_BYTES, st, x, lo_slots, g, w, bias, disp_low, hl,
                       wl, H, W, dmax, inv_q, out_disp, out_raw, tiles_x, tiles_y, ups, stat);
  else
    hipLaunchKernelGGL((k_head_final_f16<false, TH>), grid, dim3(256), T::LDS_BYTES, st, x, (size_t)0, g, w, bias, disp_low,
                       hl, wl, H, W, dmax, inv_q, out_disp, out_raw, tiles_x, tiles_y, ups, stat);
  return hipGetLastError();
}

int fuse_env() {
  static const int mode = getenv("SN_FUSE") != nullptr ? atoi(getenv("SN_FUSE")) : 4;
  return mode;
}

inline int tower_tile_width(const RefGeom& g, int nimg, int num_cu, int force_tw) {
  if (force_tw == 32 || force_tw == 64) return force_tw;
  const long wgs = 2L * num_cu;
  const long rows = (g.H + 7) / 8;
  const long r64 = ((long)((g.W + 63) / 64) * rows * nimg + wgs - 1) / wgs;
  const long r32 = ((long)((g.W + 31) / 32) * rows * nimg + wgs - 1) / wgs;
  return (double)r32 * 0.5 * 1.03 < (double)r64 ? 32 : 64;
}

hipError_t ref_conv_f16(hipStream_t st, const RefLayerF16& L, const RefGeom& g, int num_cu, int dil, const uint4* in,
                        uint4* out, const uint4* res, int nimg, bool lrelu, unsigned* tile_ctr, int force_tw = 0) {
  if (dil <= 2 && tower_tile_width(g, nimg, num_cu, force_tw) == 32) {
    if (dil == 1) return launch_ref_f16_v2<1, 32>(st, L, g, num_cu, in, out, res, nimg, lrelu, tile_ctr);
    if (dil == 2) return launch_ref_f16_v2<2, 32>(st, L, g, num_cu, in, out, res, nimg, lrelu, tile_ctr);
  }
  switch (dil) {
    case 1: return launch_ref_f16_v2<1, 64>(st, L, g, num_cu, in, out, res, nimg, lrelu, tile_ctr);
    case 2: return launch_ref_f16_v2<2, 64>(st, L, g, num_cu, in, out, res, nimg, lrelu, tile_ctr);
    case 4: return launch_ref_f16_v2<4, 32>(st, L, g, num_cu, in, out, res, nimg, lrelu, tile_ctr);
    case 8: return launch_ref_f16_v2<8, 32, 2>(st, L, g, num_cu, in, out, res, nimg, lrelu, tile_ctr);
    default: return hipErrorInvalidValue;
  }
}

hipError_t ref_block_f16(hipStream_t st, const RefLayerF16& L1, const RefLayerF16& L2, const RefGeom& g, int num_cu,
                         int dil, uint4** cur, uint4** oth, int nimg, unsigned* tile_ctr, int fuse_mode, unsigned* dump,
                         bool alt = false) {
  hipError_t e = hipErrorInvalidValue;
  bool fused = false;
  if (fuse_mode == 4 && stream_block_supports(dil)) {
    e = ref_block_stream(st, L1, L2, g, num_cu, dil, *cur, *oth, nimg, dump);
    fused = true;
  }
  if (fused) {
    uint4* t = *cur;
    *cur = *oth;
    *oth = t;
    return e;
  }
  e = ref_conv_f16(st, L1, g, num_cu, dil, *cur, *oth, nullptr, nimg, true, tile_ctr);
  if (e != hipSuccess) return e;
  RefGeom g2 = g;
  if (alt) g2.rev ^= 1;
  return ref_conv_f16(st, L2, g2, num_cu, dil, *oth, *cur, *cur, nimg, true, tile_ctr + kTileCtrStride);
}

inline bool stream_x3_supports(int dil) {
  static const bool on = !(getenv("SN_X3_STREAM") != nullptr && atoi(getenv("SN_X3_STREAM")) == 0);
  return on && (dil == 1 || dil == 2 || dil == 4 || dil == 8);
}
template <int DIL, int NWR = 2>
hipError_t launch_ref_block_stream_x3(hipStream_t st, const RefLayerF16& L1, const RefLayerF16& L2, const RefGeom& g, int num_cu,
                                      const uint4* x, uint4* y, size_t lo_slots, int nimg) {
  using T = StreamTileX3<DIL, 64, 2, 5, NWR>;
  static_assert(T::ROWS_ABOVE <= kStreamRowsAbove && T::ROWS_BELOW <= kStreamRowsBelow, "inside the zero rows the tensors are allocated with");
  auto kern = k_ref_block_stream_x3<T::DIL, T::TW, T::R, T::NXS, T::NWR>;
  hipError_t e = ensure_lds_attr(kern, T::LDS_BYTES);
  if (e != hipSuccess) return e;
  StreamSched sc;
  sc.nstrips = (g.W + T::OW - 1) / T::OW;
  sc.hsub = (g.H + DIL - 1) / DIL;
  sc.total_rows = nimg * DIL * sc.nstrips * sc.hsub;
  int nwg = num_cu;
  if (nwg > sc.total_rows) nwg = sc.total_rows;
  if (nwg < 1) nwg = 1;
  sc.rows_per_wg = (sc.total_rows + nwg - 1) / nwg;
  const int grid = (sc.total_rows + sc.rows_per_wg - 1) / sc.rows_per_wg;
  hipLaunchKernelGGL(kern, dim3(grid), dim3(128 * T::NWR), T::LDS_BYTES, st, x, y, lo_slots * 16, L1.wfrag, L1.bias, L2.wfrag,
                     L2.bias, g, sc);
  return hipGetLastError();
}
hipError_t ref_block_f16x3(hipStream_t st, const RefLayerF16& L1, const RefLayerF16& L2, const RefGeom& g, int num_cu, int dil,
                           uint4** cur, uint4** oth, size_t lo_slots, int nimg, bool stream = true) {
  if (stream && stream_x3_supports(dil)) {
    hipError_t e = hipErrorInvalidValue;
    static const int nwr = getenv("SN_X3_NWR") ? atoi(getenv("SN_X3_NWR")) : 4;
    if (nwr == 4) {
      if (dil == 1) e = launch_ref_block_stream_x3<1, 4>(st, L1, L2, g, num_cu, *cur, *oth, lo_slots, nimg);
      else if (dil == 2) e = launch_ref_block_stream_x3<2, 4>(st, L1, L2, g, num_cu, *cur, *oth, lo_slots, nimg);
      else if (dil == 4) e = launch_ref_block_stream_x3<4, 4>(st, L1, L2, g, num_cu, *cur, *oth, lo_slots, nimg);
      else e = launch_ref_block_stream_x3<8, 4>(st, L1, L2, g, num_cu, *cur, *oth, lo_slots, nimg);
    } else if (dil == 1) e = launch_ref_block_stream_x3<1>(st, L1, L2, g, num_cu, *cur, *oth, lo_slots, nimg);
    else if (dil == 2) e = launch_ref_block_stream_x3<2>(st, L1, L2, g, num_cu, *cur, *oth, lo_slots, nimg);
    else if (dil == 4) e = launch_ref_block_stream_x3<4>(st, L1, L2, g, num_cu, *cur, *oth, lo_slots, nimg);
    else e = launch_ref_block_stream_x3<8>(st, L1, L2, g, num_cu, *cur, *oth, lo_slots, nimg);
    uint4* t = *cur;
    *cur = *oth;
    *oth = t;
    return e;
  }
  hipError_t e = ref_conv_f16x3(st, L1, g, num_cu, dil, *cur, *oth, nullptr, lo_slots, nimg, true);
  if (e != hipSuccess) return e;
  return ref_conv_f16x3(st, L2, g, num_cu, dil, *oth, *cur, *cur, lo_slots, nimg, true);
}

inline int piece_pairs(const sn_handle* h, int nb, int rb) {
  int pb = h->piece > 0 ? h->piece : 16;
  if (pb > nb) pb = nb;
  if (pb < rb) pb = rb;
  return pb;
}
inline int level_chunk_pairs(int rb, int pb, int lv) {
  const long r = (long)rb << (2 * lv);
  return lv == 0 ? rb : (r < pb ? (int)r : pb);
}

int alloc_ws(sn_handle* h, Workspace* ws, int nb, int rb, int ns, int rb_x3 = 0) {
  const bool is_auto = h->precision == SN_PREC_AUTO;
  if (rb_x3 <= 0 || rb_x3 > rb) rb_x3 = rb;
  ws->nb = nb;
  ws->rb = rb;
  ws->rb_x3 = rb_x3;
  ws->ns = (ns > 1 && nb > rb) ? (ns < kMaxTowerStreams ? ns : kMaxTowerStreams) : 1;
  if (h->levels > 1) ws->ns = 1;
  ws->pb = piece_pairs(h, nb, rb);
  const int pb = ws->pb;
  const size_t HW = (size_t)h->H * h->W, HWp = (size_t)h->Hp * h->Wp, hw = (size_t)h->hl * h->wl;
  HIP_TRY(h, dalloc(&ws->in6, (size_t)nb * 6 * HW));
  bool padded_down = h->precision != SN_PREC_FP32 && down_dma_enabled();
  size_t downp_bytes[3] = {0, 0, 0};
  for (int k = h->fold_down01 ? 1 : 0; k < 3 && padded_down; ++k) {
    const SlotGeom g = down_in_geom(h->Hp >> (k + 2), h->Wp >> (k + 2));
    downp_bytes[k] = (size_t)2 * pb * 8 * g.PH * g.PW * sizeof(uint4);
    padded_down = downp_bytes[k] < ((size_t)1 << 32);
  }
  const int k_first = h->fold_down01 ? 1 : 0;
  for (int k = k_first; k < 3 && !padded_down; ++k)
    HIP_TRY(h, dalloc(&ws->down[k], (size_t)2 * pb * kC * (HWp >> (2 * (k + 1)))));
  for (int k = 0; k < 3; ++k) HIP_TRY(h, dalloc(&ws->low[k], (size_t)2 * pb * kC * hw));
  HIP_TRY(h, dalloc(&ws->feat, (size_t)2 * pb * kC * hw));
  for (int k = 0; k < 2; ++k) HIP_TRY(h, dalloc(&ws->vol[k], (size_t)pb * h->Dl * kC * hw));
  for (int k = k_first; k < 3 && padded_down; ++k) {
    HIP_TRY(h, hipMalloc(reinterpret_cast<void**>(&ws->downp[k]), downp_bytes[k]));
    HIP_TRY(h, memset_now(ws->downp[k], 0, downp_bytes[k]));
  }
  if (padded_down && feat_dma_enabled()) {
    const FeatPad g = feat_pad(h->hl, h->wl);
    const size_t bytes = (size_t)2 * pb * g.img_slots() * sizeof(uint4);
    for (int k = 0; k < 2 && bytes < ((size_t)1 << 32); ++k) {
      HIP_TRY(h, hipMalloc(reinterpret_cast<void**>(&ws->lowp[k]), bytes));
      HIP_TRY(h, memset_now(ws->lowp[k], 0, bytes));
    }
  }
  if (h->precision != SN_PREC_FP32 && agg_dma_enabled()) {
    const VolPad g = vol_pad(h->Dl, h->hl, h->wl);
    const size_t bytes = g.planes(pb) * g.plane_slots() * sizeof(uint4);
    for (int k = 0; k < 2 && bytes < ((size_t)1 << 32); ++k) {
      HIP_TRY(h, hipMalloc(reinterpret_cast<void**>(&ws->volp[k]), bytes));
      HIP_TRY(h, memset_now(ws->volp[k], 0, bytes));
    }
  }
  HIP_TRY(h, dalloc(&ws->cost, (size_t)nb * h->Dl * hw));
  HIP_TRY(h, dalloc(&ws->disp_low, (size_t)nb * hw));
  auto tensor_slots = [&](const RefGeom& rg, int pairs, int pairs_x3) {
    const size_t one = ref16_slots(rg, pairs) + ref_slack(rg), lo = ref16_slots(rg, pairs_x3) + ref_slack(rg);
    return h->precision == SN_PREC_F16X3 ? 2 * one : (is_auto ? one + lo : one);
  };
  if (h->precision == SN_PREC_FP32) {
    for (int k = 0; k < 2 * ws->ns; ++k) HIP_TRY(h, dalloc(&ws->ref[k], (size_t)rb * kC * HWp));
  } else {
    for (int k = 0; k < 2 * ws->ns; ++k)
      HIP_TRY(h, alloc_ref16(h->tw[0].rg, tensor_slots(h->tw[0].rg, rb, rb_x3), &ws->ref16_raw[k], &ws->ref16[k]));
    ws->n_chunks = (nb + rb_x3 - 1) / rb_x3 + (nb + pb - 1) / pb + 2;
    for (int lv = 1; lv < h->levels; ++lv) {
      const int rbk = level_chunk_pairs(rb_x3, pb, lv);
      ws->n_chunks += ((nb + pb - 1) / pb + 2) * ((pb + rbk - 1) / rbk + 1);
    }
    HIP_TRY(h, hipExtMallocWithFlags(reinterpret_cast<void**>(&ws->tile_ctr), kTileCtrBytes * ws->n_chunks, hipDeviceMallocFinegrained));
  }
  ws->rbk[0] = rb;
  ws->rbk_x3[0] = rb_x3;
  for (int lv = 1; lv < h->levels; ++lv) {
    const Tower& T = h->tw[lv];
    const size_t HWk = (size_t)T.Hk * T.Wk;
    ws->rbk[lv] = level_chunk_pairs(rb, pb, lv);
    ws->rbk_x3[lv] = level_chunk_pairs(rb_x3, pb, lv);
    for (int k = 0; k < 2; ++k) {
      if (h->precision == SN_PREC_FP32) {
        HIP_TRY(h, dalloc(&ws->ref_lv[lv][k], (size_t)ws->rbk[lv] * kC * HWk));
      } else {
        HIP_TRY(h, alloc_ref16(T.rg, tensor_slots(T.rg, ws->rbk[lv], ws->rbk_x3[lv]), &ws->ref16_lv_raw[lv][k], &ws->ref16_lv[lv][k]));
      }
    }
    HIP_TRY(h, dalloc(&ws->pyr[lv], (size_t)pb * 3 * HWk));
    HIP_TRY(h, dalloc(&ws->lvl_disp[lv], (size_t)pb * HWk));
  }
  HIP_TRY(h, dalloc(&ws->out_disp, (size_t)nb * HW));
  HIP_TRY(h, dalloc(&ws->out_raw, (size_t)nb * HW));
  HIP_TRY(h, dalloc(&ws->nv12, (size_t)HW * 3));
  HIP_TRY(h, dalloc(&ws->stats, kStatU64));
  HIP_TRY(h, memset_now(ws->stats, 0, kStatU64 * sizeof(unsigned long long)));
  HIP_TRY(h, hipHostMalloc(reinterpret_cast<void**>(&ws->stats_host), kStatU64 * sizeof(unsigned long long), hipHostMallocDefault));
  memset(ws->stats_host, 0, kStatU64 * sizeof(unsigned long long));
  return SN_OK;
}

void free_ws(Workspace* ws) {
  hipFree(ws->in6);
  hipFree(ws->tile_ctr);
  for (auto p : ws->down) hipFree(p);
  for (auto p : ws->low) hipFree(p);
  hipFree(ws->feat);
  for (auto p : ws->vol) hipFree(p);
  for (auto p : ws->volp) hipFree(p);
  for (auto p : ws->downp) hipFree(p);
  for (auto p : ws->lowp) hipFree(p);
  hipFree(ws->cost);
  hipFree(ws->disp_low);
  for (auto p : ws->ref) hipFree(p);
  for (auto p : ws->ref16_raw) hipFree(p);
  for (auto& lv : ws->ref_lv)
    for (auto p : lv) hipFree(p);
  for (auto& lv : ws->ref16_lv_raw)
    for (auto p : lv) hipFree(p);
  for (auto p : ws->pyr) hipFree(p);
  for (auto p : ws->lvl_disp) hipFree(p);
  hipFree(ws->out_disp);
  hipFree(ws->out_raw);
  hipFree(ws->nv12);
  hipFree(ws->stats);
  if (ws->stats_host) hipHostFree(ws->stats_host);
  *ws = Workspace();
}

int lowres_slots(sn_handle* h, Workspace& ws, hipStream_t st, int p0, int m, const int8_t* in6, bool want_cost,
                 bool prof) {
  const int Hp = h->Hp, Wp = h->Wp, hl = h->hl, wl = h->wl, Dl = h->Dl;
  const size_t HW = (size_t)h->H * h->W;
  const int8_t* in = in6 + (size_t)p0 * 6 * HW;
  const int ncu = h->num_cu, ni = 2 * m;
  auto U4 = [](float* p) { return reinterpret_cast<const uint4*>(p); };
  if (ws.downp[1] != nullptr) {
    SlotGeom gin[3];
    for (int i = 0; i < 3; ++i) gin[i] = down_in_geom(Hp >> (i + 2), Wp >> (i + 2));
    if (h->fold_down01)
      HIP_TRY(h, launch_down01(st, h->down01, in, h->H, h->W, ni, Hp / 4, Wp / 4, ws.downp[1], gin[1], ncu));
    else
      HIP_TRY(h, launch_down0_f16(st, h->down0, h->down[0].bias, in, h->H, h->W, ni, Hp / 2, Wp / 2,
                                  reinterpret_cast<float*>(ws.downp[0]), ncu, &gin[0]));
    for (int i = h->fold_down01 ? 1 : 0; i < 3; ++i) {
      const int Ho = Hp >> (i + 2), Wo = Wp >> (i + 2);
      const SlotGeom plain{Ho, Wo, 0, 0};
      const FeatPad fp = feat_pad(hl, wl);
      const SlotGeom bordered{fp.PH, fp.PW, 1, 1};
      void* const last = ws.lowp[0] ? (void*)ws.lowp[0] : (void*)ws.low[0];
      HIP_TRY(h, launch_down_dma(st, h->down[i + 1], ws.downp[i], ni, Ho, Wo, i < 2 ? (void*)ws.downp[i + 1] : last,
                                 i < 2 ? gin[i + 1] : (ws.lowp[0] ? bordered : plain), false, ncu));
    }
  } else {
  if (h->fold_down01)
    HIP_TRY(h, launch_down01(st, h->down01, in, h->H, h->W, ni, Hp / 4, Wp / 4, reinterpret_cast<uint4*>(ws.down[1]),
                             SlotGeom{Hp / 4, Wp / 4, 0, 0}, ncu));
  else
    HIP_TRY(h, launch_down0_f16(st, h->down0, h->down[0].bias, in, h->H, h->W, ni, Hp / 2, Wp / 2, ws.down[0], ncu));
  {
    float* src[3] = {ws.down[0], ws.down[1], ws.down[2]};
    float* dst[3] = {ws.down[1], ws.down[2], ws.low[0]};
    for (int i = h->fold_down01 ? 1 : 0; i < 3; ++i) {
      const int Hi = Hp >> (i + 1), Wi = Wp >> (i + 1);
      if ((h->ablate_x >> (kAblDown + i)) & 1u) HIP_TRY(h, zero_lo_slots(st, src[i], ni, (size_t)Hi * Wi));
      SlotIn ld{U4(src[i]), 0, Hi, Wi};
      HIP_TRY(h, (launch_conv_x3s<5, 2, 32, 4, 32, 32, 1, true, SlotIn>(st, h->down[i + 1], ld, ni, Hi / 2, Wi / 2, dst[i],
                                                                       nullptr, false, ncu)));
    }
  }
  }
  if (ws.lowp[0] != nullptr && ws.downp[1] != nullptr) {
    const FeatPad fp = feat_pad(hl, wl);
// ... 1669 lines not shown
  for (int ci = 0; ci < kC; ++ci)
    for (int z = 0; z < d; ++z)
      memcpy(&tmp[((size_t)z * kC + ci) * plane], &in[((size_t)ci * d + z) * plane], plane * 4);
  float *din = nullptr, *dout = nullptr;
  HIP_TRY(h, dalloc(&din, n));
  ds.track(din);
  HIP_TRY(h, dalloc(&dout, n));
  ds.track(dout);
  if (slots) {
    std::vector<_Float16> hs, ho(n * 2);
    host_to_slots(tmp.data(), d, h_px, w, hs);
    if (dma) {
      const VolPad g = vol_pad(d, h_px, w);
      const size_t phw = (size_t)g.PH * g.PW, nsl = g.planes(1) * g.plane_slots();
      std::vector<_Float16> pin(nsl * 8, (_Float16)0.f), pout(nsl * 8);
      for (size_t img = 0; img < (size_t)d * 8; ++img)
        for (int y = 0; y < h_px; ++y)
          memcpy(&pin[(((img / 8 + 1) * 8 + img % 8) * phw + (size_t)(y + 1) * g.PW + 1) * 8], &hs[(img * plane + (size_t)y * w) * 8],
                 (size_t)w * 16);
      uint4 *pdin = nullptr, *pdout = nullptr;
      HIP_TRY(h, hipMalloc(reinterpret_cast<void**>(&pdin), nsl * 16));
      ds.track(pdin);
      HIP_TRY(h, hipMalloc(reinterpret_cast<void**>(&pdout), nsl * 16));
      ds.track(pdout);
      HIP_TRY(h, hipMemcpy(pdin, pin.data(), nsl * 16, hipMemcpyHostToDevice));
      HIP_TRY(h, memset_now(pdout, 0, nsl * 16));
      HIP_TRY(h, launch_agg_dma<true>(h->stream, L, pdin, g, 1, pdout, lrelu != 0, h->num_cu));
      HIP_TRY(h, hipStreamSynchronize(h->stream));
      HIP_TRY(h, hipMemcpy(pout.data(), pdout, nsl * 16, hipMemcpyDeviceToHost));
      for (size_t img = 0; img < (size_t)d * 8; ++img)
        for (int y = 0; y < h_px; ++y)
          memcpy(&ho[(img * plane + (size_t)y * w) * 8], &pout[(((img / 8 + 1) * 8 + img % 8) * phw + (size_t)(y + 1) * g.PW + 1) * 8],
                 (size_t)w * 16);
      for (size_t i = 0; i < nsl * 8; ++i) {
        const size_t sl = i / 8, P = sl / (8 * phw), y = (sl % phw) / g.PW, x = sl % g.PW;
        const bool inside = P >= 1 && P <= (size_t)d && y >= 1 && y <= (size_t)h_px && x >= 1 && x <= (size_t)w;
        if (!inside && (float)pout[i] != 0.f) {
          set_err(h, "k_agg_x3s_dma wrote outside the image");
          return SN_ERR_DEVICE;
        }
      }
    } else {
    HIP_TRY(h, hipMemcpy(din, hs.data(), n * 4, hipMemcpyHostToDevice));
    SlotIn ls{reinterpret_cast<const uint4*>(din), d, h_px, w};
    HIP_TRY(h, (launch_conv_x3s<3, 1, 96, 8, 16, 16, 1, true, SlotIn>(h->stream, L, ls, d, h_px, w, dout, nullptr, lrelu != 0, h->num_cu)));
    HIP_TRY(h, hipStreamSynchronize(h->stream));
    HIP_TRY(h, hipMemcpy(ho.data(), dout, n * 4, hipMemcpyDeviceToHost));
    }
    host_from_slots(ho, d, h_px, w, tmp.data());
  } else {
  HIP_TRY(h, hipMemcpy(din, tmp.data(), n * 4, hipMemcpyHostToDevice));
  LoadVol3D lv{din, d, h_px, w};
  HIP_TRY(h, (launch_conv<3, 1, 1, 8, 4, 32>(h->stream, L, lv, d, h_px, w, dout, nullptr, lrelu != 0)));
  HIP_TRY(h, hipStreamSynchronize(h->stream));
  HIP_TRY(h, hipMemcpy(tmp.data(), dout, n * 4, hipMemcpyDeviceToHost));
  }
  for (int co = 0; co < kC; ++co)
    for (int z = 0; z < d; ++z)
      memcpy(&out[((size_t)co * d + z) * plane], &tmp[((size_t)z * kC + co) * plane], plane * 4);
  return SN_OK;
}

int sn_dbg_ref_conv_f16(sn_handle* h, const float* in, int h_px, int w, const float* wt, const float* bias, int dil,
                        int lrelu, const float* residual, float* out) {
  DevScope ds;
  if (!h || !in || !wt || !bias || !out || h_px <= 0 || w <= 0) return SN_ERR_ARG;
  if (dil != 1 && dil != 2 && dil != 4 && dil != 8) return SN_ERR_ARG;
  int rc = check_device(h);
  if (rc) return rc;
  const RefGeom g = make_ref_geom(h_px, w);
  const size_t slots = ref16_slots(g, 1);
  auto to_dev_layout = [&](const float* src, std::vector<_Float16>& dst) {
    dst.assign(slots * 8, (_Float16)0.f);
    for (int c = 0; c < kC; ++c)
      for (int y = 0; y < h_px; ++y)
        for (int x = 0; x < w; ++x)
          dst[((((size_t)(c >> 3)) * g.Hs + y + kRefPad) * g.Ws + x + kRefPad) * 8 + (c & 7)] =
              (_Float16)src[((size_t)c * h_px + y) * w + x];
  };
  std::vector<_Float16> hin, hres;
  to_dev_layout(in, hin);
  RefLayerF16 L;
  HostLayer hl{wt, bias, kC, kC, 9};
  if ((rc = upload_ref_f16(h, hl, &L))) return rc;
  ds.track(L.bias); ds.track(L.wfrag);
  uint4 *din = nullptr, *dout = nullptr;
  HIP_TRY(h, dalloc(&din, slots));
  ds.track(din);
  HIP_TRY(h, dalloc(&dout, slots));
  ds.track(dout);
  HIP_TRY(h, hipMemcpy(din, hin.data(), slots * 16, hipMemcpyHostToDevice));
  const uint4* dres = nullptr;
  if (residual) {
    to_dev_layout(residual, hres);
    HIP_TRY(h, hipMemcpy(dout, hres.data(), slots * 16, hipMemcpyHostToDevice));
    dres = dout;
  } else {
    HIP_TRY(h, memset_now(dout, 0, slots * 16));
  }
  unsigned* ctr = h->ws.tile_ctr;
  if (!ctr) {
    set_err(h, "sn_dbg_ref_conv_f16 needs an engine created in an fp16 mode");
    return SN_ERR_ARG;
  }
  HIP_TRY(h, hipMemsetAsync(ctr, 0, kTileCtrBytes, h->stream));
  HIP_TRY(h, ref_conv_f16(h->stream, L, g, h->num_cu, dil, din, dout, dres, 1, (lrelu & 1) != 0, ctr,
                          (lrelu & 2) ? 64 : (lrelu & 4) ? 32 : 0));
  HIP_TRY(h, hipStreamSynchronize(h->stream));
  std::vector<_Float16> hout(slots * 8);
  HIP_TRY(h, hipMemcpy(hout.data(), dout, slots * 16, hipMemcpyDeviceToHost));
  for (int c = 0; c < kC; ++c)
    for (int y = 0; y < h_px; ++y)
      for (int x = 0; x < w; ++x)
        out[((size_t)c * h_px + y) * w + x] =
            (float)hout[((((size_t)(c >> 3)) * g.Hs + y + kRefPad) * g.Ws + x + kRefPad) * 8 + (c & 7)];
  for (int c = 0; c < 4; ++c)
    for (int y = 0; y < g.Hs; ++y)
      for (int x = 0; x < g.Ws; ++x) {
        const bool inside = y >= kRefPad && y < kRefPad + h_px && x >= kRefPad && x < kRefPad + w;
        if (inside) continue;
        for (int e = 0; e < 8; ++e)
          if ((float)hout[(((size_t)c * g.Hs + y) * g.Ws + x) * 8 + e] != 0.f) {
            set_err(h, "fp16 conv wrote into the zero border");
            return SN_ERR_DEVICE;
          }
      }
  return SN_OK;
}

int sn_dbg_ref_conv_f16x3(sn_handle* h, const float* in, int h_px, int w, const float* wt, const float* bias, int dil,
                          int lrelu, const float* residual, float* out) {
  DevScope ds;
  if (!h || !in || !wt || !bias || !out || h_px <= 0 || w <= 0) return SN_ERR_ARG;
  if (dil != 1 && dil != 2 && dil != 4 && dil != 8) return SN_ERR_ARG;
  int rc = check_device(h);
  if (rc) return rc;
  const RefGeom g = make_ref_geom(h_px, w);
  const size_t lo_slots = ref16_slots(g, 1) + ref_slack(g), slots = 2 * lo_slots;
  auto idx = [&](int c, int y, int x) { return ((((size_t)(c >> 3)) * g.Hs + y + kRefPad) * g.Ws + x + kRefPad) * 8 + (c & 7); };
  auto split_to = [&](const float* src, std::vector<_Float16>& dst) {
    dst.assign(slots * 8, (_Float16)0.f);
    for (int c = 0; c < kC; ++c)
      for (int y = 0; y < h_px; ++y)
        for (int x = 0; x < w; ++x) {
          const float v = src[((size_t)c * h_px + y) * w + x];
          const _Float16 hi = (_Float16)v;
          dst[idx(c, y, x)] = hi;
          dst[lo_slots * 8 + idx(c, y, x)] = (_Float16)((v - (float)hi) * kSplitScale);
        }
  };
  std::vector<_Float16> hin, hres;
  split_to(in, hin);
  RefLayerF16 L;
  if ((rc = upload_ref_f16x3(h, HostLayer{wt, bias, kC, kC, 9}, &L))) return rc;
  ds.track(L.bias); ds.track(L.wfrag);
  uint4 *din = nullptr, *dout = nullptr;
  HIP_TRY(h, dalloc(&din, slots));
  ds.track(din);
  HIP_TRY(h, dalloc(&dout, slots));
  ds.track(dout);
  HIP_TRY(h, hipMemcpy(din, hin.data(), slots * 16, hipMemcpyHostToDevice));
  const uint4* dres = nullptr;
  if (residual) {
    split_to(residual, hres);
    HIP_TRY(h, hipMemcpy(dout, hres.data(), slots * 16, hipMemcpyHostToDevice));
    dres = dout;
  } else {
    HIP_TRY(h, memset_now(dout, 0, slots * 16));
  }
  HIP_TRY(h, ref_conv_f16x3(h->stream, L, g, h->num_cu, dil, din, dout, dres, lo_slots, 1, lrelu != 0));
  HIP_TRY(h, hipStreamSynchronize(h->stream));
  std::vector<_Float16> hout(slots * 8);
  HIP_TRY(h, hipMemcpy(hout.data(), dout, slots * 16, hipMemcpyDeviceToHost));
  for (int c = 0; c < kC; ++c)
    for (int y = 0; y < h_px; ++y)
      for (int x = 0; x < w; ++x)
        out[((size_t)c * h_px + y) * w + x] =
            (float)hout[idx(c, y, x)] + (float)hout[lo_slots * 8 + idx(c, y, x)] * kSplitInv;
  for (int part = 0; part < 2; ++part)
    for (int c = 0; c < 4; ++c)
      for (int y = 0; y < g.Hs; ++y)
        for (int x = 0; x < g.Ws; ++x) {
          if (y >= kRefPad && y < kRefPad + h_px && x >= kRefPad && x < kRefPad + w) continue;
          for (int e = 0; e < 8; ++e)
            if ((float)hout[part * lo_slots * 8 + (((size_t)c * g.Hs + y) * g.Ws + x) * 8 + e] != 0.f) {
              set_err(h, "f16x3 conv wrote into the zero border");
              return SN_ERR_DEVICE;
            }
        }
  return SN_OK;
}

int sn_dbg_ref_block_f16x3(sn_handle* h, const float* in, int h_px, int w, const float* w1, const float* b1, const float* w2,
                           const float* b2, int dil, int form, float* out) {
  DevScope ds;
  if (!h || !in || !w1 || !b1 || !w2 || !b2 || !out || h_px <= 0 || w <= 0) return SN_ERR_ARG;
  if (dil != 1 && dil != 2 && dil != 4 && dil != 8) return SN_ERR_ARG;
  if (form != 0 && form != 1) return SN_ERR_ARG;
  if (form == 1 && !stream_x3_supports(dil)) return SN_ERR_ARG;
  int rc = check_device(h);
  if (rc) return rc;
  const RefGeom g = make_ref_geom(h_px, w);
  const size_t lo_slots = ref16_slots(g, 1) + ref_slack(g), slots = 2 * lo_slots;
  auto idx = [&](int c, int y, int x) { return ((((size_t)(c >> 3)) * g.Hs + y + kRefPad) * g.Ws + x + kRefPad) * 8 + (c & 7); };
  std::vector<_Float16> hin(slots * 8, (_Float16)0.f);
  for (int c = 0; c < kC; ++c)
    for (int y = 0; y < h_px; ++y)
      for (int x = 0; x < w; ++x) {
        const float v = in[((size_t)c * h_px + y) * w + x];
        const _Float16 hi = (_Float16)v;
        hin[idx(c, y, x)] = hi;
        hin[lo_slots * 8 + idx(c, y, x)] = (_Float16)((v - (float)hi) * kSplitScale);
      }
  RefLayerF16 L1, L2;
  if ((rc = upload_ref_f16x3(h, HostLayer{w1, b1, kC, kC, 9}, &L1))) return rc;
  ds.track(L1.bias); ds.track(L1.wfrag);
  if ((rc = upload_ref_f16x3(h, HostLayer{w2, b2, kC, kC, 9}, &L2))) return rc;
  ds.track(L2.bias); ds.track(L2.wfrag);
  uint4 *da = nullptr, *db = nullptr, *da_raw = nullptr, *db_raw = nullptr;
  HIP_TRY(h, alloc_ref16(g, slots, &da_raw, &da));
  ds.track(da_raw);
  HIP_TRY(h, alloc_ref16(g, slots, &db_raw, &db));
  ds.track(db_raw);
  HIP_TRY(h, hipMemcpy(da, hin.data(), slots * 16, hipMemcpyHostToDevice));
  uint4 *cur = da, *oth = db;
  HIP_TRY(h, ref_block_f16x3(h->stream, L1, L2, g, h->num_cu, dil, &cur, &oth, lo_slots, 1, form == 1));
  HIP_TRY(h, hipStreamSynchronize(h->stream));
  std::vector<_Float16> hout(slots * 8);
  HIP_TRY(h, hipMemcpy(hout.data(), cur, slots * 16, hipMemcpyDeviceToHost));
  for (int c = 0; c < kC; ++c)
    for (int y = 0; y < h_px; ++y)
      for (int x = 0; x < w; ++x)
        out[((size_t)c * h_px + y) * w + x] = (float)hout[idx(c, y, x)] + (float)hout[lo_slots * 8 + idx(c, y, x)] * kSplitInv;
  for (int part = 0; part < 2; ++part)
    for (int c = 0; c < 4; ++c)
      for (int y = 0; y < g.Hs; ++y)
        for (int x = 0; x < g.Ws; ++x) {
          if (y >= kRefPad && y < kRefPad + h_px && x >= kRefPad && x < kRefPad + w) continue;
          for (int e = 0; e < 8; ++e)
            if ((float)hout[part * lo_slots * 8 + (((size_t)c * g.Hs + y) * g.Ws + x) * 8 + e] != 0.f) {
              set_err(h, "f16x3 residual block wrote into the zero border");
              return SN_ERR_DEVICE;
            }
        }
  return SN_OK;
}

int sn_dbg_ref_block_f16(sn_handle* h, const float* in, int h_px, int w, const float* w1, const float* b1,
                         const float* w2, const float* b2, int dil, float* out) {
  DevScope ds;
  if (!h || !in || !w1 || !b1 || !w2 || !b2 || !out || h_px <= 0 || w <= 0) return SN_ERR_ARG;
  const int form = dil >> 8;
  if (form != 0 && form != 2) return SN_ERR_ARG;
  const int fuse_mode = form == 2 ? 4 : 0;
  dil &= 0xff;
  if (dil != 1 && dil != 2 && dil != 4 && dil != 8) return SN_ERR_ARG;
  if (fuse_mode == 4 && !stream_block_supports(dil)) return SN_ERR_ARG;
  int rc = check_device(h);
  if (rc) return rc;
  const RefGeom g = make_ref_geom(h_px, w);
  const size_t slots = ref16_slots(g, 1);
  auto idx = [&](int c, int y, int x) { return ((((size_t)(c >> 3)) * g.Hs + y + kRefPad) * g.Ws + x + kRefPad) * 8 + (c & 7); };
  std::vector<_Float16> hin(slots * 8, (_Float16)0.f);
  for (int c = 0; c < kC; ++c)
    for (int y = 0; y < h_px; ++y)
      for (int x = 0; x < w; ++x) hin[idx(c, y, x)] = (_Float16)in[((size_t)c * h_px + y) * w + x];
  RefLayerF16 L1, L2;
  if ((rc = upload_ref_f16(h, HostLayer{w1, b1, kC, kC, 9}, &L1))) return rc;
  ds.track(L1.bias); ds.track(L1.wfrag);
  if ((rc = upload_ref_f16(h, HostLayer{w2, b2, kC, kC, 9}, &L2))) return rc;
  ds.track(L2.bias); ds.track(L2.wfrag);
  uint4 *da = nullptr, *db = nullptr, *da_raw = nullptr, *db_raw = nullptr;
  HIP_TRY(h, alloc_ref16(g, slots + ref_slack(g), &da_raw, &da));
  ds.track(da_raw);
  HIP_TRY(h, alloc_ref16(g, slots + ref_slack(g), &db_raw, &db));
  ds.track(db_raw);
  HIP_TRY(h, hipMemcpy(da, hin.data(), slots * 16, hipMemcpyHostToDevice));
  uint4 *cur = da, *oth = db;
  if (!h->ws.tile_ctr) {
    set_err(h, "sn_dbg_ref_block_f16 needs an engine created in an fp16 mode");
    return SN_ERR_ARG;
  }
  HIP_TRY(h, hipMemsetAsync(h->ws.tile_ctr, 0, kTileCtrBytes, h->stream));
  HIP_TRY(h, ref_block_f16(h->stream, L1, L2, g, h->num_cu, dil, &cur, &oth, 1, h->ws.tile_ctr, fuse_mode, h->dump));
  HIP_TRY(h, hipStreamSynchronize(h->stream));
  std::vector<_Float16> hout(slots * 8);
  HIP_TRY(h, hipMemcpy(hout.data(), cur, slots * 16, hipMemcpyDeviceToHost));
  for (int c = 0; c < kC; ++c)
    for (int y = 0; y < h_px; ++y)
      for (int x = 0; x < w; ++x) out[((size_t)c * h_px + y) * w + x] = (float)hout[idx(c, y, x)];
  for (int c = 0; c < 4; ++c)
    for (int y = 0; y < g.Hs; ++y)
      for (int x = 0; x < g.Ws; ++x) {
        if (y >= kRefPad && y < kRefPad + h_px && x >= kRefPad && x < kRefPad + w) continue;
        for (int e = 0; e < 8; ++e)
          if ((float)hout[(((size_t)c * g.Hs + y) * g.Ws + x) * 8 + e] != 0.f) {
            set_err(h, "fp16 residual block wrote into the zero border");
            return SN_ERR_DEVICE;
          }
      }
  return SN_OK;
}

int sn_dbg_ref_tail_f16(sn_handle* h, int n, const float* in, int hk, int wk, const float* w1, const float* b1, const float* w2,
                        const float* b2, const float* head_w, float head_b, const float* low, int ups, float dnorm, int h_out,
                        int w_out, int form, float* out_disp, int32_t* out_raw) {
  DevScope ds;
  if (!h || !in || !w1 || !b1 || !w2 || !b2 || !head_w || !low || !out_disp || !out_raw) return SN_ERR_ARG;
  if (n <= 0 || hk <= 0 || wk <= 0 || h_out <= 0 || w_out <= 0 || h_out > hk || w_out > wk || (ups != 16 && ups != 2) ||
      hk % ups || wk % ups || (form != 0 && form != 1) || !(dnorm > 0.f))
    return SN_ERR_ARG;
  if (h->precision != SN_PREC_F16 && h->precision != SN_PREC_AUTO) {
    set_err(h, "sn_dbg_ref_tail_f16 needs an engine created with SN_PREC_F16 or SN_PREC_AUTO");
    return SN_ERR_ARG;
  }
  int rc = check_device(h);
  if (rc) return rc;
  const RefGeom g = make_ref_geom(hk, wk);
  const size_t per = ref16_slots(g, 1), slots = ref16_slots(g, n);
  if ((slots + ref_slack(g) + ref_front(g)) * 16 >= ((size_t)1 << 32)) return SN_ERR_ARG;
  std::vector<_Float16> hin(slots * 8, (_Float16)0.f);
  for (int i = 0; i < n; ++i)
    for (int c = 0; c < kC; ++c)
      for (int y = 0; y < hk; ++y) {
        const float* src = in + (((size_t)i * kC + c) * hk + y) * wk;
        _Float16* dst = &hin[(i * per + (((size_t)(c >> 3)) * g.Hs + y + kRefPad) * g.Ws + kRefPad) * 8 + (c & 7)];
        for (int x = 0; x < wk; ++x) dst[(size_t)x * 8] = (_Float16)src[x];
      }
  RefLayerF16 L1, L2;
  HeadLayer hd;
  rc = upload_ref_f16(h, HostLayer{w1, b1, kC, kC, 9}, &L1);
  ds.track(L1.bias); ds.track(L1.wfrag);
  if (rc) return rc;
  rc = upload_ref_f16(h, HostLayer{w2, b2, kC, kC, 9}, &L2);
  ds.track(L2.bias); ds.track(L2.wfrag);
  if (rc) return rc;
  rc = upload_head(h, HostLayer{head_w, &head_b, 1, kC, 9}, &hd);
  ds.track(hd.w);
  if (rc) return rc;
  uint4 *da = nullptr, *db = nullptr, *da_raw = nullptr, *db_raw = nullptr;
  HIP_TRY(h, alloc_ref16(g, slots + ref_slack(g), &da_raw, &da));
  ds.track(da_raw);
  HIP_TRY(h, alloc_ref16(g, slots + ref_slack(g), &db_raw, &db));
  ds.track(db_raw);
  HIP_TRY(h, hipMemcpy(da, hin.data(), slots * 16, hipMemcpyHostToDevice));
  const int sh = hk / ups, sw = wk / ups;
  const size_t nlow = (size_t)n * sh * sw, nout = (size_t)n * h_out * w_out;
  float *dlow = nullptr, *dd = nullptr;
  int32_t* dr = nullptr;
  HIP_TRY(h, dalloc(&dlow, nlow));
  ds.track(dlow);
  HIP_TRY(h, dalloc(&dd, nout));
  ds.track(dd);
  HIP_TRY(h, dalloc(&dr, nout));
  ds.track(dr);
  HIP_TRY(h, hipMemcpy(dlow, low, nlow * 4, hipMemcpyHostToDevice));
  HIP_TRY(h, memset_now(dd, 0xff, nout * 4));
  HIP_TRY(h, memset_now(dr, 0xff, nout * 4));
  const float inv_q = (float)(1.0 / (kWireFactor * (double)kOutScale));
  const UpScale us{1.0f / (float)ups, (float)ups};
  if (form == 1) {
    StreamHeadArgs ha{hd.w, dlow, dd, dr, hd.bias, dnorm, inv_q, sh, sw, h_out, w_out, us};
    HIP_TRY(h, ref_block_stream_tail(h->stream, L1, L2, g, h->num_cu, da, n, h->dump, ha));
  } else {
    HIP_TRY(h, ref_block_stream(h->stream, L1, L2, g, h->num_cu, 1, da, db, n, h->dump));
    HIP_TRY(h, launch_head_final_f16(h->stream, false, db, 0, g, hd.w, hd.bias, dlow, sh, sw, h_out, w_out, dnorm, inv_q, us, dd, dr, n));
  }
  HIP_TRY(h, hipStreamSynchronize(h->stream));
  HIP_TRY(h, hipMemcpy(out_disp, dd, nout * 4, hipMemcpyDeviceToHost));
  HIP_TRY(h, hipMemcpy(out_raw, dr, nout * 4, hipMemcpyDeviceToHost));
  return SN_OK;
}

__global__ __launch_bounds__(256) void k_depth_from_raw(const int32_t* __restrict__ raw, size_t n, float scale, float fB,
                                                        float* __restrict__ depth, float* __restrict__ disp) {
  for (size_t i = (size_t)blockIdx.x * 256 + threadIdx.x; i < n; i += (size_t)gridDim.x * 256) {
    const float dis = (float)raw[i] * scale;
    depth[i] = (float)((double)fB / ((double)dis * 16.0 * 12.0) / 1000.0);
    if (disp) disp[i] = dis * 16.0f * 12.0f;
  }
}

int sn_depth_from_raw(sn_handle* h, int n, const int32_t* raw, float focal_px, float baseline_mm, float* depth_m, float* disp_px,
                      int mem, void* stream) {
  if (!h || !raw || !depth_m || n <= 0 || n > h->max_batch || (mem != SN_MEM_HOST && mem != SN_MEM_DEVICE)) return SN_ERR_ARG;
  int rc = check_device(h);
  if (rc) return rc;
  const size_t cnt = (size_t)n * h->H * h->W;
  hipStream_t st = stream ? static_cast<hipStream_t>(stream) : h->stream;
  const float fB = focal_px * baseline_mm;
  const int32_t* draw = raw;
  float *ddepth = depth_m, *ddisp = disp_px;
  DevScope ds;
  if (mem == SN_MEM_HOST) {
    int32_t* a = nullptr;
    float *b = nullptr, *c = nullptr;
    HIP_TRY(h, dalloc(&a, cnt));
    ds.track(a);
    HIP_TRY(h, dalloc(&b, cnt));
    ds.track(b);
    if (disp_px) {
      HIP_TRY(h, dalloc(&c, cnt));
      ds.track(c);
    }
    HIP_TRY(h, hipMemcpyAsync(a, raw, cnt * 4, hipMemcpyHostToDevice, st));
    draw = a;
    ddepth = b;
    ddisp = c;
  }
  unsigned grid = (unsigned)((cnt + 255) / 256);
  if (grid > 4096) grid = 4096;
  hipLaunchKernelGGL(k_depth_from_raw, dim3(grid), dim3(256), 0, st, draw, cnt, kOutScale, fB, ddepth, ddisp);
  HIP_TRY(h, hipGetLastError());
  if (mem == SN_MEM_HOST) {
    HIP_TRY(h, hipMemcpyAsync(depth_m, ddepth, cnt * 4, hipMemcpyDeviceToHost, st));
    if (disp_px) HIP_TRY(h, hipMemcpyAsync(disp_px, ddisp, cnt * 4, hipMemcpyDeviceToHost, st));
    HIP_TRY(h, hipStreamSynchronize(st));
  }
  return SN_OK;
}

__global__ __launch_bounds__(256) void k_copy_limited(uint4* __restrict__ dst, const uint4* __restrict__ src, size_t n16) {
  for (size_t i = (size_t)blockIdx.x * 256 + threadIdx.x; i < n16; i += (size_t)gridDim.x * 256) dst[i] = src[i];
}

int sn_dbg_copy_limited(void* dst, const void* src, size_t bytes, int workgroups, void* stream) {
  if (!dst || !src || (bytes & 15) || workgroups <= 0 || workgroups > 65535 || ((uintptr_t)dst & 15) || ((uintptr_t)src & 15)) return SN_ERR_ARG;
  hipLaunchKernelGGL(k_copy_limited, dim3((unsigned)workgroups), dim3(256), 0, static_cast<hipStream_t>(stream),
                     static_cast<uint4*>(dst), static_cast<const uint4*>(src), bytes / 16);
  return hipGetLastError() == hipSuccess ? SN_OK : SN_ERR_DEVICE;
}

int sn_dbg_read(sn_handle* h, const char* what, float* dst, size_t cap, size_t* n) {
  if (!h || !what || !n) return SN_ERR_ARG;
  int rc = check_device(h);
  if (rc) return rc;
  const size_t hw = (size_t)h->hl * h->wl;
  const float* src = nullptr;
  size_t cnt = 0;
  if (!strcmp(what, "stream_prio")) {
    *n = 1;
    if (dst && cap >= 1) dst[0] = h->stream_prio ? 1.f : 0.f;
    return (dst && cap < 1) ? SN_ERR_ARG : SN_OK;
  }
  if (!strcmp(what, "feat_l")) { src = h->ws.feat; cnt = kC * hw; }
  else if (!strcmp(what, "feat_r")) { src = h->ws.feat + kC * hw; cnt = kC * hw; }
  else if (!strcmp(what, "cost")) { src = h->ws.cost; cnt = h->Dl * hw; }
  else if (!strcmp(what, "disp_low")) { src = h->ws.disp_low; cnt = hw; }
  else if (!strcmp(what, "tile_ctr") && h->ws.tile_ctr) { src = reinterpret_cast<const float*>(h->ws.tile_ctr); cnt = kTileCtrBytes / 4 * h->ws.n_chunks; }
  else if (!strcmp(what, "refine_x") && h->precision == SN_PREC_FP32) { src = h->ws.ref[0]; cnt = (size_t)kC * h->Hp * h->Wp; }
  else if (!strncmp(what, "level", 5) && what[5] >= '1' && what[5] < '0' + h->levels && what[6] == 0) {
    const int k = what[5] - '0';
    src = h->ws.lvl_disp[k];
    cnt = (size_t)h->tw[k].Hk * h->tw[k].Wk;
  }
  else return SN_ERR_ARG;
  *n = cnt;
  if (!dst) return SN_OK;
  if (cap < cnt) return SN_ERR_ARG;
  HIP_TRY(h, hipStreamSynchronize(h->stream));
  HIP_TRY(h, hipMemcpy(dst, src, cnt * 4, hipMemcpyDeviceToHost));
  return SN_OK;
}

}
```

include/stereonet_hip.h:

```cpp
#ifndef STEREONET_HIP_H_
#define STEREONET_HIP_H_

#include <stddef.h>
#include <stdint.h>

#ifdef __cplusplus
extern "C" {
#endif

typedef struct sn_handle sn_handle;

#define SN_ABI_VERSION 3
int sn_abi_version(void);

enum {
  SN_OK = 0,
  SN_ERR_ARG = -1,
  SN_ERR_FILE = -2,
  SN_ERR_FORMAT = -3,
  SN_ERR_DEVICE = -4,
  SN_ERR_NOMEM = -5,
  SN_ERR_BUSY = -6,
  SN_ERR_TICKET = -7
};

enum { SN_MEM_HOST = 0, SN_MEM_DEVICE = 1 };

enum {
  SN_PREC_DEFAULT = 0,
  SN_PREC_F16X3 = 1,
  SN_PREC_F16 = 2,
  SN_PREC_FP32 = 3,
  SN_PREC_AUTO = 4
};

typedef struct sn_config {
  int device;
  int max_batch;
  int width;
  int height;
  int dmax;
  int precision;
  int task_num;
  int refine_chunk;
  int piece;
} sn_config;

typedef struct sn_io_info {
  int width, height, dmax;
  int in_channels;
  int max_batch, precision, task_num, device;
  float out_scale;
  size_t in_bytes;
  size_t out_bytes;
  double flops_per_pair;
  int refine_chunk;
  int piece;
  int tower_streams;
  int refine_levels;
  int precision_selected;
} sn_io_info;

int sn_create(const char *model_file, const sn_config *cfg, sn_handle **out);
int sn_destroy(sn_handle *h);
int sn_get_io_info(const sn_handle *h, sn_io_info *info);
const char *sn_strerror(int code);
const char *sn_last_error(const sn_handle *h);

typedef struct sn_refine_stats {
  int levels;
  int precision;
  int precision_selected;
  int precision_last;
  uint64_t calls, pairs;
  uint64_t switches;
  uint64_t reruns;
  double level_px[4];
  double residual_px;
  double running_px;
  double envelope_px;
  double limit_px;
  double selfcheck_epe_px;
  double selfcheck_residual_px;
} sn_refine_stats;
int sn_get_refine_stats(sn_handle *h, sn_refine_stats *out);

#define SN_AUTO_BUDGET_PX 0.85e-3
#define SN_AUTO_ENVELOPE_CAP 4.0
#define SN_AUTO_REENTRY 0.8
#define SN_AUTO_CALM_CALLS 8
typedef struct sn_auto_state {
  int mode;
  int calm;
  double envelope_px;
  double epe_per_px;
  double running_px;
  uint64_t switches;
} sn_auto_state;
double sn_auto_envelope_px(int refine_levels);
int sn_auto_init(sn_auto_state *s, int refine_levels);
double sn_auto_limit_px(const sn_auto_state *s);
int sn_auto_observe(sn_auto_state *s, double residual_px);

int sn_infer_i8(sn_handle *h, const int8_t *in_nchw6, int32_t *out_i32, float *out_disp,
                int mem, void *stream);
int sn_infer_batch(sn_handle *h, int n, const int8_t *in_nchw6, int32_t *out_i32, float *out_disp,
                   int mem, void *stream);

int sn_preprocess_nv12(sn_handle *h, const uint8_t *left_nv12, const uint8_t *right_nv12,
                       int w, int h_px, int8_t *out_nchw6, int mem, void *stream);
int sn_infer_sbs_nv12(sn_handle *h, const uint8_t *sbs_nv12, int w2, int h_px, int32_t *out_i32,
                      float *out_disp, int8_t *out_tensor, int mem, void *stream);

int sn_preprocess_sbs_nv12_batch(sn_handle *h, int n, const uint8_t *sbs_nv12, int w2, int h_px, int8_t *out_nchw6,
                                 int mem, void *stream);

int sn_submit(sn_handle *h, const int8_t *in_nchw6_host, int32_t *out_i32_host, float *out_disp_host,
              int timeout_ms, uint64_t *ticket);
int sn_submit_nv12(sn_handle *h, const uint8_t *sbs_nv12_host, int w2, int h_px, int32_t *out_i32_host,
                   float *out_disp_host, int timeout_ms, uint64_t *ticket);
int sn_wait(sn_handle *h, uint64_t ticket, float *infer_ms);
int sn_synchronize(sn_handle *h);

typedef struct sn_mgpu sn_mgpu;
int sn_mgpu_shard(int n, int ndev, int k, int *first, int *count);
int sn_mgpu_create(const char *model_file, const sn_config *cfg, const int *devices, int ndev, sn_mgpu **out);
int sn_mgpu_destroy(sn_mgpu *m);
int sn_mgpu_get_info(const sn_mgpu *m, int *ndev, int *per_device_batch, int *gather_kind );
int sn_mgpu_get_handle(sn_mgpu *m, int k, sn_handle **h);
int sn_mgpu_infer_batch(sn_mgpu *m, int n, const int8_t *in_nchw6_host, int32_t *out_i32_host, float *out_disp_host);
int sn_mgpu_infer_batch_device(sn_mgpu *m, int n, const int8_t *const *in_per_device, int32_t *out_i32_root,
                               float *out_disp_root);
int sn_mgpu_submit_device(sn_mgpu *m, int n, const int8_t *const *in_per_device, int32_t *out_i32_root,
                          float *out_disp_root, uint64_t *ticket);
int sn_mgpu_wait(sn_mgpu *m, uint64_t ticket);
const char *sn_mgpu_last_error(const sn_mgpu *m);
#define SN_MGPU_SLOTS 2
typedef struct sn_mgpu_ring {
  uint64_t next;
  uint64_t slot_ticket[SN_MGPU_SLOTS];
} sn_mgpu_ring;
int sn_mgpu_ring_init(sn_mgpu_ring *r);
int sn_mgpu_ring_submit(sn_mgpu_ring *r, uint64_t *ticket, int *slot);
int sn_mgpu_ring_wait(sn_mgpu_ring *r, uint64_t ticket, int *slot);

enum {
  SN_STAGE_FEATURES = 0,
  SN_STAGE_AGGREGATE = 1,
  SN_STAGE_REFINE = 2,
  SN_STAGE_REFINE_CONV = 3,
  SN_STAGE_TOTAL = 4,
  SN_STAGE_DOMINANT = 5,
  SN_STAGE_COUNT = 6
};
int sn_set_profiling(sn_handle *h, int enable);
int sn_get_stage_ms(sn_handle *h, float *ms, int count);
int sn_get_dominant_kernel(sn_handle *h, char *name, size_t name_cap, int *launches,
                           double *flops_per_launch, double *bytes_per_launch);

int sn_dbg_conv2d(sn_handle *h, const float *in, int cin, int h_px, int w, const float *wt,
                  const float *bias, int k, int stride, int dil, int lrelu, const float *residual,
                  float *out);
int sn_dbg_down0(sn_handle *h, const int8_t *in6, int h_px, int w, const float *wt, const float *bias, int tc,
                 float *out);
int sn_dbg_round_kernels_f16(const float *w, int nkernels, float *out);
int sn_dbg_compose_down01(const float *w0, const float *b0, const float *w1, const float *b1, float *weff,
                          float *beff);
int sn_dbg_down01(sn_handle *h, const int8_t *in6, int h_px, int w, const float *w0, const float *b0,
                  const float *w1, const float *b1, float *out);
int sn_dbg_refin(sn_handle *h, const float *disp_low, const int8_t *in6, int h_px, int w, int dmax,
                 const float *wt, const float *bias, int split, float *out);
int sn_dbg_conv3d(sn_handle *h, const float *in, int d, int h_px, int w, const float *wt,
                  const float *bias, int lrelu, float *out);
int sn_dbg_ref_conv_f16(sn_handle *h, const float *in, int h_px, int w, const float *wt, const float *bias,
                        int dil, int lrelu, const float *residual, float *out);
int sn_dbg_ref_conv_f16x3(sn_handle *h, const float *in, int h_px, int w, const float *wt, const float *bias,
                          int dil, int lrelu, const float *residual, float *out);
int sn_dbg_ref_block_f16(sn_handle *h, const float *in, int h_px, int w, const float *w1, const float *b1,
                         const float *w2, const float *b2, int dil, float *out);
int sn_dbg_ref_block_f16x3(sn_handle *h, const float *in, int h_px, int w, const float *w1, const float *b1,
                           const float *w2, const float *b2, int dil, int form, float *out);
int sn_dbg_ref_tail_f16(sn_handle *h, int n, const float *in, int hk, int wk, const float *w1, const float *b1,
                        const float *w2, const float *b2, const float *head_w, float head_b, const float *low, int ups,
                        float dnorm, int h_out, int w_out, int form, float *out_disp, int32_t *out_raw);
int sn_dbg_read(sn_handle *h, const char *what, float *dst, size_t cap, size_t *n);
int sn_depth_from_raw(sn_handle *h, int n, const int32_t *raw, float focal_px, float baseline_mm, float *depth_m,
                      float *disp_px, int mem, void *stream);

int sn_dbg_copy_limited(void *dst, const void *src, size_t bytes, int workgroups, void *stream);

#ifdef __cplusplus
}
#endif
#endif
```

Measured before the change: 3059.

## Pack images into a shared strip space for streamed residual blocks

New measurement: 3070 (median of 6 runs). No clear change (+0.4%).

```diff
diff --git a/hobot_stereonet_amd/api.py b/hobot_stereonet_amd/api.py
--- a/hobot_stereonet_amd/api.py
+++ b/hobot_stereonet_amd/api.py
@@ -108,6 +108,7 @@
     lib.sn_dbg_ref_conv_f16.argtypes = [vp, fp, ip, ip, fp, fp, ip, ip, fp, fp]
     lib.sn_dbg_ref_conv_f16x3.argtypes = [vp, fp, ip, ip, fp, fp, ip, ip, fp, fp]
     lib.sn_dbg_ref_block_f16.argtypes = [vp, fp, ip, ip, fp, fp, fp, fp, ip, fp]
+    lib.sn_dbg_ref_block_stream_f16.argtypes = [vp, ip, fp, ip, ip, fp, fp, fp, fp, ip, ip, fp]
     lib.sn_dbg_ref_block_f16x3.argtypes = [vp, fp, ip, ip, fp, fp, fp, fp, ip, ip, fp]
     lib.sn_dbg_ref_tail_f16.argtypes = [vp, ip, fp, ip, ip, fp, fp, fp, fp, fp, C.c_float, fp, ip, C.c_float, ip, ip, ip, fp, i32p]
     lib.sn_dbg_read.argtypes = [vp, C.c_char_p, fp, C.c_size_t, C.POINTER(C.c_size_t)]
@@ -124,7 +125,7 @@
                  "sn_infer_sbs_nv12", "sn_preprocess_sbs_nv12_batch", "sn_submit", "sn_submit_nv12", "sn_wait", "sn_synchronize", "sn_set_profiling",
                  "sn_get_stage_ms", "sn_get_dominant_kernel", "sn_mgpu_shard", "sn_mgpu_create", "sn_mgpu_destroy",
                  "sn_mgpu_get_info", "sn_mgpu_get_handle", "sn_mgpu_infer_batch", "sn_mgpu_infer_batch_device",
-                 "sn_mgpu_submit_device", "sn_mgpu_wait", "sn_mgpu_ring_init", "sn_mgpu_ring_submit", "sn_mgpu_ring_wait", "sn_dbg_conv2d", "sn_dbg_down0", "sn_dbg_compose_down01", "sn_dbg_round_kernels_f16", "sn_dbg_down01", "sn_dbg_refin", "sn_dbg_conv3d", "sn_dbg_ref_conv_f16", "sn_dbg_ref_conv_f16x3", "sn_dbg_ref_block_f16", "sn_dbg_ref_block_f16x3", "sn_dbg_ref_tail_f16", "sn_dbg_read", "sn_dbg_copy_limited", "sn_depth_from_raw", "sn_get_refine_stats", "sn_auto_init", "sn_auto_observe"):
+                 "sn_mgpu_submit_device", "sn_mgpu_wait", "sn_mgpu_ring_init", "sn_mgpu_ring_submit", "sn_mgpu_ring_wait", "sn_dbg_conv2d", "sn_dbg_down0", "sn_dbg_compose_down01", "sn_dbg_round_kernels_f16", "sn_dbg_down01", "sn_dbg_refin", "sn_dbg_conv3d", "sn_dbg_ref_conv_f16", "sn_dbg_ref_conv_f16x3", "sn_dbg_ref_block_f16", "sn_dbg_ref_block_stream_f16", "sn_dbg_ref_block_f16x3", "sn_dbg_ref_tail_f16", "sn_dbg_read", "sn_dbg_copy_limited", "sn_depth_from_raw", "sn_get_refine_stats", "sn_auto_init", "sn_auto_observe"):
         getattr(lib, name).restype = C.c_int
     _lib = lib
     return lib
@@ -419,6 +420,15 @@
                     "sn_dbg_ref_block_f16")
         return out
 
+    def dbg_ref_block_stream_f16(self, x, w1, b1, w2, b2, dil=1, pack=1):
+        a = [np.ascontiguousarray(v, np.float32) for v in (x, w1, b1, w2, b2)]
+        n, _, h, w = a[0].shape
+        out = np.empty((n, 32, h, w), np.float32)
+        self._check(self._lib.sn_dbg_ref_block_stream_f16(self._h, n, a[0].ctypes.data, h, w, a[1].ctypes.data,
+                                                          a[2].ctypes.data, a[3].ctypes.data, a[4].ctypes.data, dil,
+                                                          int(pack), out.ctypes.data), "sn_dbg_ref_block_stream_f16")
+        return out
+
     def dbg_ref_block_f16x3(self, x, w1, b1, w2, b2, dil=1, streamed=False):
         a = [np.ascontiguousarray(v, np.float32) for v in (x, w1, b1, w2, b2)]
         _, h, w = a[0].shape
diff --git a/hobot_stereonet_amd/csrc/sn_stream_block.hpp b/hobot_stereonet_amd/csrc/sn_stream_block.hpp
--- a/hobot_stereonet_amd/csrc/sn_stream_block.hpp
+++ b/hobot_stereonet_amd/csrc/sn_stream_block.hpp
@@ -23,20 +23,21 @@
 
 namespace sn {
 
-template <int DIL_, int TW_ = 64, int R_ = 4, int NXS_ = 6, int NWR_ = 4, bool HEAD_ = false>
+template <int DIL_, int TW_ = 64, int R_ = 4, int NXS_ = 6, int NWR_ = 4, bool HEAD_ = false, bool PACK_ = false>
 struct StreamTile {
-  static constexpr bool HEAD = HEAD_;
+  static constexpr bool HEAD = HEAD_, PACK = PACK_;
+  static constexpr int CDIL = PACK_ ? 1 : DIL_;
   static constexpr int DIL = DIL_, TW = TW_, R = R_, NXS = NXS_, NTS = 3, PF = NXS_ - (HEAD_ ? 3 : 4);
   static constexpr int NWR = NWR_;
   static constexpr int HS = HEAD_ ? 1 : 0;
-  static constexpr int YW = TW - 2 * DIL;
+  static constexpr int YW = TW - 2 * CDIL;
   static constexpr int OW = YW - 2 * HS;
-  static constexpr int X0OFF = -HS;
+  static constexpr int X0OFF = PACK_ ? 1 : -HS;
   static constexpr int LAG = HEAD_ ? 3 : 2;
   static constexpr int PROWS = 2 * R + 2;
   static constexpr int PRING_BYTES = HEAD_ ? PROWS * 9 * TW * 4 : 0;
   static constexpr int WIN_BYTES = HEAD_ ? NWR_ * 2 * 64 * 4 : 0;
-  static constexpr int XW = TW + 2 * DIL;
+  static constexpr int XW = TW + 2 * CDIL;
   static constexpr int CSEG = TW / 32;
   static constexpr int SPW = R * CSEG / NWR;
   static constexpr int XROW = 4 * XW, TROW = 4 * TW;
@@ -50,6 +51,7 @@
   static constexpr int LDS_BYTES = (XRING + TRING) * 16 + 2 * 2 * 16 * 4 + PRING_BYTES + WIN_BYTES;
   static constexpr int ROWS_ABOVE = (R + HS) * DIL, ROWS_BELOW = (R + 2 + HS) * DIL - 1;
   static_assert(!HEAD_ || (DIL_ == 1 && R_ == 4 && TW_ == 64 && NWR_ == 4), "the tail form is written for the dilation-1 strip shape");
+  static_assert(!(HEAD_ && PACK_), "the tail form keeps the per-image strips");
   static_assert(SPW == 1 || SPW == 2, "segments per wave");
   static_assert(CSEG % SPW == 0, "a wave's segments lie in one row");
   static_assert(PF == 2, "prefetch distance the counted waits are written for");
@@ -62,7 +64,51 @@
   int hsub;
   int total_rows;
   int rows_per_wg;
+  int nimg;
 };
+
+struct PackCol {
+  unsigned slot;
+  bool ok;
+};
+template <int DIL>
+__device__ __forceinline__ PackCol pack_col(int v, const RefGeom& g, int nimg) {
+  const int pitch = g.W + DIL;
+  int o = v - 1;
+  int img = o >= 0 ? o / pitch : 0;
+  bool ok = o >= 0 && img < nimg;
+  img = img < nimg ? img : nimg - 1;
+  o -= img * pitch;
+  int col;
+  if constexpr (DIL == 1) {
+    col = o;
+    ok = ok && o < g.W;
+  } else {
+    const int a = g.W / DIL, b = g.W - a * DIL;
+    const int lb = b * (a + 2);
+    int p, sc, n;
+    if (o < lb) {
+      p = o / (a + 2);
+      sc = o - p * (a + 2);
+      n = a + 1;
+    } else {
+      const int o2 = o - lb;
+      const int pp = o2 / (a + 1);
+      sc = o2 - pp * (a + 1);
+      p = b + pp;
+      n = a;
+    }
+    ok = ok && sc < n;
+    col = p + sc * DIL;
+  }
+  if (!ok) col = -1;
+  return PackCol{(unsigned)img * 4u * (unsigned)g.Hs * (unsigned)g.Ws + (unsigned)(col + kRefPad), ok};
+}
+
+__device__ __forceinline__ int xcd_band_share(int b, int n) {
+  const int x = b & 7, q = n >> 3, r = n & 7;
+  return x * q + (x < r ? x : r) + (b >> 3);
+}
 
 template <int R, int HS = 0>
 struct StreamIter {
@@ -175,13 +221,13 @@
   unsigned long long* stat = nullptr;
 };
 
-template <int DIL, int TW, int R, int NXS, int NWR, bool HEAD = false>
+template <int DIL, int TW, int R, int NXS, int NWR, bool HEAD = false, bool PACK = false>
 __global__ __launch_bounds__(128 * NWR, NWR / 2) __attribute__((amdgpu_waves_per_eu(NWR / 2, NWR / 2))) void k_ref_block_stream_f16(const uint4* __restrict__ xin, uint4* __restrict__ yout,
                                                                 const uint4* __restrict__ wfrag1, const float* __restrict__ bias1,
                                                                 const uint4* __restrict__ wfrag2, const float* __restrict__ bias2,
                                                                 RefGeom g, StreamSched sc, uint4* __restrict__ dump, StreamHeadArgs ha) {
-  using T = StreamTile<DIL, TW, R, NXS, NWR, HEAD>;
-  constexpr int HS = T::HS;
+  using T = StreamTile<DIL, TW, R, NXS, NWR, HEAD, PACK>;
+  constexpr int HS = T::HS, CDIL = T::CDIL;
   extern __shared__ __attribute__((aligned(16))) uint4 lds[];
   uint4* const xring = lds;
   uint4* const tring = lds + T::XRING;
@@ -193,7 +239,7 @@
   const int j = lane & 31, gh = lane >> 5;
   const int role = wave / NWR, rw = wave % NWR;
 
-  const int f0 = (int)blockIdx.x * sc.rows_per_wg;
+  const int f0 = (PACK ? xcd_band_share((int)blockIdx.x, (int)gridDim.x) : (int)blockIdx.x) * sc.rows_per_wg;
   int f1 = f0 + sc.rows_per_wg;
   if (f1 > sc.total_rows) f1 = sc.total_rows;
   if (f0 >= f1) return;
@@ -209,7 +255,7 @@
   auto decode_sp = [&](int sp, int& img, int& py, int& x0) {
     const int t = sp / sc.nstrips;
     x0 = (sp - t * sc.nstrips) * T::OW + T::X0OFF;
-    img = t / DIL;
+    img = PACK ? 0 : t / DIL;
     py = t - img * DIL;
   };
   const unsigned plane_b = (unsigned)g.Hs * (unsigned)g.Ws * 16u;
@@ -243,24 +289,33 @@
     constexpr int KWMAX = T::KW;
     const int kw = (T::NINST - rw + NWR - 1) / NWR;
     unsigned dma_voff[KWMAX];
-#pragma unroll
-    for (int k = 0; k < KWMAX; ++k) {
-      const int i = rw + NWR * k;
-      int s = i * 64 + lane;
-      s = s < T::XGROUP ? s : T::XGROUP - 1;
-      const int r = s / T::XROW;
-      const int rem = s - r * T::XROW;
-      const int blk = rem / T::XW;
-      const int c = rem - blk * T::XW;
-      dma_voff[k] = (unsigned)blk * plane_b + ((unsigned)(r * DIL) * (unsigned)g.Ws + (unsigned)c) * 16u;
-    }
+    auto dma_lanes = [&](int x0) {
+#pragma unroll
+      for (int k = 0; k < KWMAX; ++k) {
+        const int i = rw + NWR * k;
+        int s = i * 64 + lane;
+        s = s < T::XGROUP ? s : T::XGROUP - 1;
+        const int r = s / T::XROW;
+        const int rem = s - r * T::XROW;
+        const int blk = rem / T::XW;
+        const int c = rem - blk * T::XW;
+        const unsigned col = PACK ? pack_col<DIL>(x0 - 2 + c, g, sc.nimg).slot : (unsigned)c;
+        dma_voff[k] = (unsigned)blk * plane_b + ((unsigned)(r * DIL) * (unsigned)g.Ws + col) * 16u;
+      }
+    };
+    if constexpr (!PACK) dma_lanes(0);
     long last_base = 0;
     auto dma_issue = [&](const StreamIter<R, HS>& it, int grp) {
       if (it.live) {
         int img, py, x0;
         decode_sp(it.sp, img, py, x0);
         const int row = (it.v0 - HS - R + R * it.j) * DIL + py;
-        last_base = (((long)img * 4 * g.Hs + (row + kRefPad)) * (long)g.Ws + (x0 - 2 * DIL + kRefPad)) * 16;
+        if constexpr (PACK) {
+          if (it.j == 0) dma_lanes(x0);
+          last_base = (long)(row + kRefPad) * (long)g.Ws * 16;
+        } else {
+          last_base = (((long)img * 4 * g.Hs + (row + kRefPad)) * (long)g.Ws + (x0 - 2 * DIL + kRefPad)) * 16;
+        }
       }
       const char* src = reinterpret_cast<const char*>(xin) + last_base;
       const unsigned dst = lds_addr(xring + grp * T::XGP);
@@ -291,6 +346,10 @@
     block_barrier();
 
     int c1_py = 0, c1_x0 = 0;
+    bool c1_tok[T::SPW];
+    bool c1_cols = true;
+#pragma unroll
+    for (int s = 0; s < T::SPW; ++s) c1_tok[s] = true;
     int qx = 0, qt = 0;
     for (int q = 0; q < nss; ++q) {
       dm.step(q + 2, 0, f0, f1, sc.hsub);
@@ -372,6 +431,15 @@
         if (c1.j == 1) {
           int img;
           decode_sp(c1.sp, img, c1_py, c1_x0);
+          if constexpr (PACK) {
+            bool all = true;
+#pragma unroll
+            for (int s = 0; s < T::SPW; ++s) {
+              c1_tok[s] = pack_col<DIL>(c1_x0 - 1 + (cseg0 + s) * 32 + j, g, sc.nimg).ok;
+              all = all && c1_tok[s];
+            }
+            c1_cols = __builtin_amdgcn_ballot_w64(!all) == 0;
+          }
         }
         const uint4* xp[3];
 #pragma unroll
@@ -381,12 +449,12 @@
         }
         const f32x16 bv = *reinterpret_cast<const f32x16*>(s_bias + gh * 16);
         f32x16 acc[T::SPW];
-        stream_conv36<DIL, T::XW, T::SPW>(xp, wf, bv, acc);
+        stream_conv36<CDIL, T::XW, T::SPW>(xp, wf, bv, acc);
         SN_STAMP(2);
         const int trow = (c1.v0 - HS - 1 + R * (c1.j - 1) + rowW) * DIL + c1_py;
         const bool row_ok = trow >= 0 && trow < g.H;
         const int tc0 = c1_x0 - DIL;
-        const bool interior = row_ok && tc0 >= 0 && tc0 + TW <= g.W;
+        const bool interior = row_ok && (PACK ? c1_cols : tc0 >= 0 && tc0 + TW <= g.W);
         uint4* tw = tring + qt * T::TGP + rowW * T::TROW + lane_w;
         auto write_t = [&](auto is_interior) {
 #pragma unroll
@@ -394,7 +462,7 @@
             bool inside = true;
             if (!decltype(is_interior)::value) {
               const int c = tc0 + (cseg0 + s) * 32 + j;
-              inside = row_ok && c >= 0 && c < g.W;
+              inside = row_ok && (PACK ? c1_tok[s] : c >= 0 && c < g.W);
             }
             unsigned pk[4][2];
 #pragma unroll
@@ -425,12 +493,12 @@
     SN_STAMP_WG(1);
   } else {
     const int lane_t = gh * T::TW + cseg0 * 32 + j;
-    const int lane_y = 2 * DIL + cseg0 * 32 + j;
+    const int lane_y = 2 * CDIL + cseg0 * 32 + j;
     block_barrier();
 
     StreamIter<R, HS> c2, ep;
     c2.live = ep.live = 0;
-    half8 ah[2], al[2];
+    half8 ah[2];
     uint2 rres[T::SPW][4];
     int p4 = 0;
     if constexpr (HEAD) {
@@ -438,10 +506,10 @@
       for (int kk = 0; kk < 2; ++kk)
 #pragma unroll
         for (int e = 0; e < 8; ++e) {
-          const float wv = j < 9 ? ha.w[(16 * kk + 8 * gh + e) * 9 + j] : 0.f;
+          const int tap = j < 16 ? j : j - 16;
+          const float wv = tap < 9 ? ha.w[(16 * kk + 8 * gh + e) * 9 + tap] : 0.f;
           const _Float16 hi = (_Float16)wv;
-          ah[kk][e] = hi;
-          al[kk][e] = (_Float16)((wv - (float)hi) * kSplitScale);
+          ah[kk][e] = j < 16 ? hi : (_Float16)((wv - (float)hi) * kSplitScale);
         }
 #pragma unroll
       for (int s = 0; s < T::SPW; ++s)
@@ -450,6 +518,13 @@
     }
     int ep_img = 0, ep_py = 0, ep_x0 = 0;
     const unsigned lane_o = (unsigned)(cseg0 * 32 + j) * 16u + (unsigned)(2 * gh) * plane_b;
+    unsigned ep_off[T::SPW];
+    bool ep_ok[T::SPW];
+#pragma unroll
+    for (int s = 0; s < T::SPW; ++s) {
+      ep_off[s] = 0u;
+      ep_ok[s] = false;
+    }
     f32x16 acc[T::SPW];
 #pragma unroll
     for (int s = 0; s < T::SPW; ++s)
@@ -465,7 +540,18 @@
       const int gt1 = qt >= 1 ? qt - 1 : qt - 1 + T::NTS, gt2 = qt >= 2 ? qt - 2 : qt - 2 + T::NTS;
       SN_STAMP(0);
       if (doe) {
-        if (ep.j == 1) decode_sp(ep.sp, ep_img, ep_py, ep_x0);
+        if (ep.j == 1) {
+          decode_sp(ep.sp, ep_img, ep_py, ep_x0);
+          if constexpr (PACK) {
+#pragma unroll
+            for (int s = 0; s < T::SPW; ++s) {
+              const int c = (cseg0 + s) * 32 + j;
+              const PackCol pc = pack_col<DIL>(ep_x0 + c, g, sc.nimg);
+              ep_off[s] = pc.slot * 16u + (unsigned)(2 * gh) * plane_b;
+              ep_ok[s] = c < T::OW && pc.ok;
+            }
+          }
+        }
         const int sub = ep.v0 - HS - 2 + R * (ep.j - 1) + rowW;
         const int row = sub * DIL + ep_py;
         if constexpr (HEAD) {
@@ -492,12 +578,9 @@
                 pk[qd][1] = ok ? pk[qd][1] : 0u;
               }
             }
-            f32x16 a0, a1;
-#pragma unroll
-            for (int r = 0; r < 16; ++r) {
-              a0[r] = 0.f;
-              a1[r] = 0.f;
-            }
+            f32x16 a0;
+#pragma unroll
+            for (int r = 0; r < 16; ++r) a0[r] = 0.f;
 #pragma unroll
             for (int kk = 0; kk < 2; ++kk) {
               const auto r0 = __builtin_amdgcn_permlane32_swap(pk[2 * kk][0], pk[2 * kk + 1][0], false, false);
@@ -505,19 +588,19 @@
               const uint4 sl = uint4{r0[0], r1[0], r0[1], r1[1]};
               const half8 xh = *reinterpret_cast<const half8*>(&sl);
               a0 = __builtin_amdgcn_mfma_f32_32x32x16_f16(ah[kk], xh, a0, 0, 0, 0);
-              a1 = __builtin_amdgcn_mfma_f32_32x32x16_f16(al[kk], xh, a1, 0, 0, 0);
             }
             float* dst = pring + prow * (9 * TW) + (cseg0 + s) * 32 + j;
 #pragma unroll
-            for (int r = 0; r < 4; ++r) dst[(4 * gh + r) * TW] = a0[r] + a1[r] * kSplitInv;
-            if (gh == 0) dst[8 * TW] = a0[4] + a1[4] * kSplitInv;
+            for (int r = 0; r < 4; ++r) dst[(4 * gh + r) * TW] = a0[r] + a0[r + 8] * kSplitInv;
+            if (gh == 0) dst[8 * TW] = a0[4] + a0[12] * kSplitInv;
           }
         } else
         if (sub >= ep.v0 && sub < ep.v1 && row < g.H) {
           const int rr = rowW - 2;
           const uint4* xrow = xring + (rr < 0 ? gx3 : gx2) * T::XGP + (rr & (R - 1)) * T::XROW + lane_y;
-          const unsigned ob = (((unsigned)ep_img * 4u * (unsigned)g.Hs + (unsigned)(row + kRefPad)) * (unsigned)g.Ws +
-                               (unsigned)(ep_x0 + kRefPad)) * 16u;
+          const unsigned ob = PACK ? (unsigned)(row + kRefPad) * (unsigned)g.Ws * 16u
+                                   : (((unsigned)ep_img * 4u * (unsigned)g.Hs + (unsigned)(row + kRefPad)) * (unsigned)g.Ws +
+                                      (unsigned)(ep_x0 + kRefPad)) * 16u;
 #pragma unroll
           for (int s = 0; s < T::SPW; ++s) {
             unsigned pk[4][2];
@@ -536,7 +619,15 @@
               sl[k] = uint4{r0[0], r1[0], r0[1], r1[1]};
             }
             const int c = (cseg0 + s) * 32 + j;
-            if (c < T::OW && ep_x0 + c < g.W) {
+            if constexpr (PACK) {
+              if (ep_ok[s]) {
+#pragma unroll
+                for (int k = 0; k < 2; ++k) {
+                  char* o = reinterpret_cast<char*>(yout) + (ob + (unsigned)k * plane_b);
+                  *reinterpret_cast<uint4*>(o + ep_off[s]) = sl[k];
+                }
+              }
+            } else if (c < T::OW && ep_x0 + c < g.W) {
 #pragma unroll
               for (int k = 0; k < 2; ++k) {
                 char* o = reinterpret_cast<char*>(yout) + (ob + (unsigned)k * plane_b + (unsigned)s * 512u);
@@ -565,7 +656,7 @@
           tp[ky] = tring + (rr < 0 ? gt2 : gt1) * T::TGP + (rr & (R - 1)) * T::TROW + lane_t;
         }
         const f32x16 bv = *reinterpret_cast<const f32x16*>(s_bias + (2 + gh) * 16);
-        stream_conv36<DIL, T::TW, T::SPW>(tp, wf, bv, acc);
+        stream_conv36<CDIL, T::TW, T::SPW>(tp, wf, bv, acc);
       }
       SN_STAMP(2);
       asm volatile("s_waitcnt lgkmcnt(0)" ::: "memory");
diff --git a/hobot_stereonet_amd/csrc/stereonet_hip.hip b/hobot_stereonet_amd/csrc/stereonet_hip.hip
--- a/hobot_stereonet_amd/csrc/stereonet_hip.hip
+++ b/hobot_stereonet_amd/csrc/stereonet_hip.hip
@@ -786,6 +786,10 @@
 using StreamTile2 = StreamTile<2, 64, 4, 6, 4>;
 using StreamTile4 = StreamTile<4, 128, 2, 6, 4>;
 using StreamTile8 = StreamTile<8, 128, 2, 6, 4>;
+using StreamTile1P = StreamTile<1, 64, 4, 6, 4, false, true>;
+using StreamTile2P = StreamTile<2, 64, 4, 6, 4, false, true>;
+using StreamTile4P = StreamTile<4, 128, 2, 6, 4, false, true>;
+using StreamTile8P = StreamTile<8, 128, 2, 6, 4, false, true>;
 using StreamTileTail = StreamTile<1, 64, 4, 5, 4, true>;
 static_assert(StreamTileTail::ROWS_ABOVE <= kRefPad && StreamTileTail::ROWS_BELOW <= StreamTile8::ROWS_BELOW, "tail form stays inside the zero rows");
 constexpr int cmax4(int a, int b, int c, int d) { return (a > b ? a : b) > (c > d ? c : d) ? (a > b ? a : b) : (c > d ? c : d); }
@@ -794,6 +798,9 @@
 constexpr int kRefSlackRows = kStreamRowsBelow - kRefPad + 1;
 constexpr int kRefFrontRows = (kStreamRowsAbove > kRefPad ? kStreamRowsAbove - kRefPad : 0) + 1;
 static_assert(kRefSlackRows == 24 && kRefFrontRows == 9, "zero rows around the fp16 tower tensors follow the StreamTile list");
+static_assert(cmax4(StreamTile1P::ROWS_ABOVE, StreamTile2P::ROWS_ABOVE, StreamTile4P::ROWS_ABOVE, StreamTile8P::ROWS_ABOVE) <= kStreamRowsAbove &&
+              cmax4(StreamTile1P::ROWS_BELOW, StreamTile2P::ROWS_BELOW, StreamTile4P::ROWS_BELOW, StreamTile8P::ROWS_BELOW) <= kStreamRowsBelow,
+              "the packed strips stay inside the same zero rows");
 size_t ref_slack(const RefGeom& g) {
   const size_t rows = (size_t)kRefSlackRows * g.Ws;
   return rows > 4096 ? rows : 4096;
@@ -964,16 +971,22 @@
 hipError_t launch_ref_block_stream(hipStream_t st, const RefLayerF16& L1, const RefLayerF16& L2, const RefGeom& g, int num_cu,
                                    const uint4* x, uint4* y, int nimg, unsigned* dump, const StreamHeadArgs& ha = StreamHeadArgs{}) {
   constexpr int DIL = T::DIL;
-  auto kern = k_ref_block_stream_f16<T::DIL, T::TW, T::R, T::NXS, T::NWR, T::HEAD>;
+  auto kern = k_ref_block_stream_f16<T::DIL, T::TW, T::R, T::NXS, T::NWR, T::HEAD, T::PACK>;
   if (dump == nullptr) return hipErrorInvalidValue;
   hipError_t e = ensure_lds_attr(kern, T::LDS_BYTES);
   if (e != hipSuccess) return e;
   StreamSched sc;
   const int Wn = T::HEAD ? ha.W : g.W, Hn = T::HEAD ? ha.H : g.H;
   if (T::HEAD && (!ha.w || !ha.disp_low || (!ha.out_disp && !ha.out_raw) || ha.W > g.W || ha.H > g.H || ha.ups.rs > 0.5f)) return hipErrorInvalidValue;
-  sc.nstrips = (Wn + T::OW - 1) / T::OW;
   sc.hsub = (Hn + DIL - 1) / DIL;
-  sc.total_rows = nimg * DIL * sc.nstrips * sc.hsub;
+  sc.nimg = nimg;
+  if (T::PACK) {
+    sc.nstrips = (nimg * (Wn + DIL) - 1 + T::OW - 1) / T::OW;
+    sc.total_rows = DIL * sc.nstrips * sc.hsub;
+  } else {
+    sc.nstrips = (Wn + T::OW - 1) / T::OW;
+    sc.total_rows = nimg * DIL * sc.nstrips * sc.hsub;
+  }
   static const int wg_env = getenv("SN_STREAM_WGS") ? atoi(getenv("SN_STREAM_WGS")) : 0;
   int nwg = wg_env > 0 ? wg_env : num_cu;
   if (nwg > sc.total_rows) nwg = sc.total_rows;
@@ -990,8 +1003,23 @@
   return launch_ref_block_stream<StreamTileTail>(st, L1, L2, g, num_cu, x, nullptr, nimg, dump, ha);
 }
 
+inline bool stream_pack_dil(int dil) {
+  static const int mode = getenv("SN_STREAM_PACK") != nullptr ? atoi(getenv("SN_STREAM_PACK")) : 1;
+  return mode == 2 || (mode == 1 && dil == 1);
+}
+
 hipError_t ref_block_stream(hipStream_t st, const RefLayerF16& L1, const RefLayerF16& L2, const RefGeom& g, int num_cu, int dil,
-                            const uint4* x, uint4* y, int nimg, unsigned* dump) {
+                            const uint4* x, uint4* y, int nimg, unsigned* dump, int pack = -1) {
+  if (pack < 0) pack = stream_pack_dil(dil) ? 1 : 0;
+  if (pack) {
+    switch (dil) {
+      case 1: return launch_ref_block_stream<StreamTile1P>(st, L1, L2, g, num_cu, x, y, nimg, dump);
+      case 2: return launch_ref_block_stream<StreamTile2P>(st, L1, L2, g, num_cu, x, y, nimg, dump);
+      case 4: return launch_ref_block_stream<StreamTile4P>(st, L1, L2, g, num_cu, x, y, nimg, dump);
+      case 8: return launch_ref_block_stream<StreamTile8P>(st, L1, L2, g, num_cu, x, y, nimg, dump);
+      default: return hipErrorInvalidValue;
+    }
+  }
   switch (dil) {
     case 1: return launch_ref_block_stream<StreamTile1>(st, L1, L2, g, num_cu, x, y, nimg, dump);
     case 2: return launch_ref_block_stream<StreamTile2>(st, L1, L2, g, num_cu, x, y, nimg, dump);
@@ -3267,6 +3295,66 @@
   return SN_OK;
 }
 
+int sn_dbg_ref_block_stream_f16(sn_handle* h, int n, const float* in, int h_px, int w, const float* w1, const float* b1,
+                                const float* w2, const float* b2, int dil, int pack, float* out) {
+  DevScope ds;
+  if (!h || !in || !w1 || !b1 || !w2 || !b2 || !out || n <= 0 || h_px <= 0 || w <= 0 || (pack != 0 && pack != 1)) return SN_ERR_ARG;
+  if (dil != 1 && dil != 2 && dil != 4 && dil != 8) return SN_ERR_ARG;
+  if (!h->ws.tile_ctr) {
+    set_err(h, "sn_dbg_ref_block_stream_f16 needs an engine created in an fp16 mode");
+    return SN_ERR_ARG;
+  }
+  int rc = check_device(h);
+  if (rc) return rc;
+  const RefGeom g = make_ref_geom(h_px, w);
+  const size_t per = ref16_slots(g, 1), slots = ref16_slots(g, n);
+  if ((slots + ref_slack(g) + ref_front(g)) * 16 >= ((size_t)1 << 32)) return SN_ERR_ARG;
+  std::vector<_Float16> hin(slots * 8, (_Float16)0.f);
+  for (int i = 0; i < n; ++i)
+    for (int c = 0; c < kC; ++c)
+      for (int y = 0; y < h_px; ++y) {
+        const float* src = in + (((size_t)i * kC + c) * h_px + y) * w;
+        _Float16* dst = &hin[(i * per + (((size_t)(c >> 3)) * g.Hs + y + kRefPad) * g.Ws + kRefPad) * 8 + (c & 7)];
+        for (int x = 0; x < w; ++x) dst[(size_t)x * 8] = (_Float16)src[x];
+      }
+  RefLayerF16 L1, L2;
+  rc = upload_ref_f16(h, HostLayer{w1, b1, kC, kC, 9}, &L1);
+  ds.track(L1.bias); ds.track(L1.wfrag);
+  if (rc) return rc;
+  rc = upload_ref_f16(h, HostLayer{w2, b2, kC, kC, 9}, &L2);
+  ds.track(L2.bias); ds.track(L2.wfrag);
+  if (rc) return rc;
+  uint4 *da = nullptr, *db = nullptr, *da_raw = nullptr, *db_raw = nullptr;
+  HIP_TRY(h, alloc_ref16(g, slots + ref_slack(g), &da_raw, &da));
+  ds.track(da_raw);
+  HIP_TRY(h, alloc_ref16(g, slots + ref_slack(g), &db_raw, &db));
+  ds.track(db_raw);
+  HIP_TRY(h, hipMemcpy(da, hin.data(), slots * 16, hipMemcpyHostToDevice));
+  HIP_TRY(h, ref_block_stream(h->stream, L1, L2, g, h->num_cu, dil, da, db, n, h->dump, pack));
+  HIP_TRY(h, hipStreamSynchronize(h->stream));
+  std::vector<_Float16> hout(slots * 8);
+  HIP_TRY(h, hipMemcpy(hout.data(), db, slots * 16, hipMemcpyDeviceToHost));
+  for (int i = 0; i < n; ++i)
+    for (int c = 0; c < kC; ++c)
+      for (int y = 0; y < h_px; ++y) {
+        float* dst = out + (((size_t)i * kC + c) * h_px + y) * w;
+        const _Float16* src = &hout[(i * per + (((size_t)(c >> 3)) * g.Hs + y + kRefPad) * g.Ws + kRefPad) * 8 + (c & 7)];
+        for (int x = 0; x < w; ++x) dst[x] = (float)src[(size_t)x * 8];
+      }
+  for (int i = 0; i < n; ++i)
+    for (int c = 0; c < 4; ++c)
+      for (int y = 0; y < g.Hs; ++y)
+        for (int x = 0; x < g.Ws; ++x) {
+          if (y >= kRefPad && y < kRefPad + h_px && x >= kRefPad && x < kRefPad + w) continue;
+          for (int e = 0; e < 8; ++e)
+            if ((float)hout[(i * per + ((size_t)c * g.Hs + y) * g.Ws + x) * 8 + e] != 0.f) {
+              set_err(h, "streamed residual block wrote into the zero border");
+              return SN_ERR_DEVICE;
+            }
+        }
+  return SN_OK;
+}
+
 int sn_dbg_ref_tail_f16(sn_handle* h, int n, const float* in, int hk, int wk, const float* w1, const float* b1, const float* w2,
                         const float* b2, const float* head_w, float head_b, const float* low, int ups, float dnorm, int h_out,
                         int w_out, int form, float* out_disp, int32_t* out_raw) {
diff --git a/include/stereonet_hip.h b/include/stereonet_hip.h
--- a/include/stereonet_hip.h
+++ b/include/stereonet_hip.h
@@ -178,6 +178,8 @@
                           int dil, int lrelu, const float *residual, float *out);
 int sn_dbg_ref_block_f16(sn_handle *h, const float *in, int h_px, int w, const float *w1, const float *b1,
                          const float *w2, const float *b2, int dil, float *out);
+int sn_dbg_ref_block_stream_f16(sn_handle *h, int n, const float *in, int h_px, int w, const float *w1, const float *b1,
+                                const float *w2, const float *b2, int dil, int pack, float *out);
 int sn_dbg_ref_block_f16x3(sn_handle *h, const float *in, int h_px, int w, const float *w1, const float *b1,
                            const float *w2, const float *b2, int dil, int form, float *out);
 int sn_dbg_ref_tail_f16(sn_handle *h, int n, const float *in, int hk, int wk, const float *w1, const float *b1,
```
